# rockcarry/ffcnn

Measured on AMD Instinct MI355X. Metric: frames/sec yolo-fastest-1.1 @320x320 batch-64 per GPU (u8 BGR frames -> net_input's conversion in the first kernel -> full forward: conv stack + YOLO decode + NMS, boxes on rank 0), higher is better.
Workload: dtype f32

## Files before the change

### ffcnn_amd/capi.py

```python
import ctypes as C
import os
import subprocess

import numpy as np

HERE = os.path.dirname(os.path.abspath(__file__))
ROOT = os.path.dirname(HERE)
DATA = os.path.join(ROOT, "data")
CFG = os.path.join(DATA, "yolo-fastest-1.1.cfg")
WEIGHTS = os.path.join(DATA, "yolo-fastest-1.1.weights")

f32p = C.POINTER(C.c_float)


class FFGPU:
    MAX_DET = 128
    MERGE_LDS_SLOTS = 1024
    KEEP_ALL, COMPAT_V6, NO_GRAPH, NO_FUSE, HOST_DETS, SPLIT2, CONCURRENT, BF16_PW = 1, 2, 4, 8, 16, 32, 64, 128
    FEAT_FLAT, FEAT_MEAN, FEAT_MAX = 0, 1, 2
    POST_NONE, POST_SOFTMAX, POST_L2 = 0, 1, 2
    TOPK_MAX = 16
    RELABEL_KEEP_SCORE, RELABEL_LABEL_SCORE = 0, 1
    RELABEL_ENTRIES, RELABEL_MERGED = 0, 1
    K_AUTO, K_GENERIC, K_DW_STREAM, K_DW_LDS, K_PW_MFMA, K_PW_GEMM, _K6, K_DENSE_SMALL, K_IGEMM, K_PW_BF16, K_GROUP_THIN, K_PW_X3, K_CONV_X3, K_PW_X3T = range(14)
# ... 226 lines not shown
ZONES_EVENTS_HEADER = ("considered", "known", "fresh", "refused", "duplicate", "anonymous", "dropped", "freed", "live", "frame")
ZONES_STATE_HEADER = 144
TRACK_DETS = 128
TRACK_ENTRIES, TRACK_MERGED = 0, 1
TRACK_IDS_HEADER = ("considered", "matched", "born", "refused", "dropped", "freed", "live", "frame")
CROP_F32, CROP_U8 = 0, 1
CROP_ENTRIES, CROP_MERGED = 0, 1
REDACT_FILL, REDACT_MOSAIC = 0, 1
REDACT_OUTSIDE = 1
REDACT_ENTRIES, REDACT_MERGED = 0, 1
BLUR_OUTSIDE = 1
BLUR_ENTRIES, BLUR_MERGED = 0, 1
DRAW_ENTRIES, DRAW_MERGED = 0, 1
YUV_BT601_LIMITED, YUV_BT601_FULL, YUV_BT709_LIMITED, YUV_BT709_FULL = 0, 1, 2, 3

assert C.sizeof(LAYER) == 120 and C.sizeof(NET) == 104 and C.sizeof(BBOX) == 24
assert C.sizeof(FrameDets) == 16 + 24 * FFGPU.MAX_DET
assert C.sizeof(BgrFrame) == 24 and C.sizeof(Nv12Frame) == 40 and C.sizeof(Tile) == 16 and C.sizeof(TileRect) == 16
assert C.sizeof(DrawStyle) == 24 and C.sizeof(CropSpec) == 72 and C.sizeof(Crop) == 48
assert C.sizeof(TrackSpec) == 32 and C.sizeof(Track) == 48
assert C.sizeof(FeatureSpec) == 16 and C.sizeof(Label) == 8 and C.sizeof(RelabelSpec) == 16
assert C.sizeof(Gallery) == 40 and C.sizeof(RedactSpec) == 40 and C.sizeof(BlurSpec) == 40
assert C.sizeof(TextItem) == 64 and C.sizeof(CaptionSpec) == 48
assert C.sizeof(SegItem) == 32 and C.sizeof(OutlineSpec) == 40
assert C.sizeof(TrailPoint) == 12 and C.sizeof(TrailSlot) == 416 and C.sizeof(TrailsSpec) == 64
assert C.sizeof(HeatSpec) == 56 and C.sizeof(HeatBlendSpec) == 48
assert C.sizeof(MotionSpec) == 64
assert C.sizeof(Zone) == 96 and C.sizeof(Line) == 32 and C.sizeof(Scene) == 1040 and C.sizeof(ZonesSpec) == 32 and C.sizeof(ZoneSlot) == 64

BOX_DTYPE = np.dtype([("type", "<i4"), ("score", "<f4"), ("x1", "<f4"), ("y1", "<f4"), ("x2", "<f4"), ("y2", "<f4")])
DETS_DTYPE = np.dtype([("count", "<i4"), ("ncand", "<i4"), ("overflow", "<i4"), ("nfull", "<i4"),
                       ("box", BOX_DTYPE, (FFGPU.MAX_DET,))])
CROP_DTYPE = np.dtype([("target", "<i4"), ("box", "<i4"), ("type", "<i4"), ("score", "<f4"), ("x0", "<i4"), ("y0", "<i4"), ("w", "<i4"), ("h", "<i4"),
                       ("sw", "<i4"), ("sh", "<i4"), ("s1", "<i4"), ("s2", "<i4")])
TRACK_DTYPE = np.dtype([("id", "<i4"), ("type", "<i4"), ("score", "<f4"), ("x1", "<f4"), ("y1", "<f4"), ("x2", "<f4"), ("y2", "<f4"),
                        ("hits", "<i4"), ("missed", "<i4"), ("born", "<i4"), ("det", "<i4"), ("reserved", "<i4")])
ZONE_SLOT_DTYPE = np.dtype([("id", "<i4"), ("px", "<f4"), ("py", "<f4"), ("inside", "<i4"), ("last", "<i4"), ("reserved", "<i4", (3,)), ("since", "<i4", (8,))])
TRAIL_POINT_DTYPE = np.dtype([("x", "<i4"), ("y", "<i4"), ("frame", "<i4")])
TRAIL_SLOT_DTYPE = np.dtype([("id", "<i4"), ("last", "<i4"), ("n", "<i4"), ("head", "<i4"), ("cx", "<i4"), ("cy", "<i4"), ("reserved", "<i4", (2,)),
                             ("ring", TRAIL_POINT_DTYPE, (32,))])
LABEL_DTYPE = np.dtype([("index", "<i4"), ("value", "<f4")])
TEXT_ITEM_DTYPE = np.dtype([("x", "<i4"), ("y", "<i4"), ("fg", "u1", (4,)), ("bg", "u1", (4,)), ("scale", "u1"), ("flags", "u1"), ("len", "u1"), ("reserved", "u1"),
                            ("text", "u1", (44,))])
SEG_ITEM_DTYPE = np.dtype([("x0", "<i4"), ("y0", "<i4"), ("x1", "<i4"), ("y1", "<i4"), ("color", "u1", (4,)), ("thickness", "u1"), ("dash", "u1"), ("flags", "u1"),
                           ("reserved", "u1"), ("reserved2", "<i4", (2,))])

EXPORTS = ["net_load", "net_free", "net_input", "net_forward", "net_dump", "net_profile", "groupconv",
           "ffgpu_device_count", "ffgpu_set_device", "ffgpu_last_error", "ffgpu_build_info",
           "ffgpu_net_weights_dev", "ffgpu_net_weights_commit",
           "ffgpu_exec_create", "ffgpu_exec_destroy", "ffgpu_exec_batch", "ffgpu_exec_arena_bytes",
           "ffgpu_exec_kernel_count", "ffgpu_exec_work_model", "ffgpu_exec_set_scale", "ffgpu_exec_forward_dev", "ffgpu_exec_forward_host",
           "ffgpu_exec_forward_bgr_dev", "ffgpu_exec_forward_bgr_frames_dev", "ffgpu_exec_forward_nv12_frames_dev", "ffgpu_exec_dets_dev", "ffgpu_exec_dets_host", "ffgpu_exec_set_ring", "ffgpu_exec_set_ring_strided", "ffgpu_exec_read_dets", "ffgpu_exec_read_layer", "ffgpu_exec_hash_layers",
           "ffgpu_exec_read_boxes", "ffgpu_exec_cand_capacity", "ffgpu_exec_graph_captures",
           "ffgpu_exec_profile", "ffgpu_exec_profile_steps", "ffgpu_exec_step_model", "ffgpu_groupconv_dev", "ffgpu_groupconv_kernel_name", "ffgpu_groupconv_time_dev", "ffgpu_irb_dev", "ffgpu_irb_flags_dev", "ffgpu_irb_plan_text", "ffgpu_irb_thin_launch_text", "ffgpu_irb_s2_launch_text", "ffgpu_irb_stage_plan_text", "ffgpu_front_plan_text", "ffgpu_irb_instantiations", "ffgpu_knobs_text", "ffgpu_dwpw_dev", "ffgpu_packed_records_bytes", "ffgpu_pack_records", "ffgpu_unpack_records",
           "ffgpu_shard_range", "ffgpu_node_create", "ffgpu_node_destroy", "ffgpu_node_ndev", "ffgpu_node_shard", "ffgpu_node_set_scale",
           "ffgpu_node_input_dev", "ffgpu_node_input_slot_dev", "ffgpu_node_depth", "ffgpu_node_rccl_ranks", "ffgpu_node_forward", "ffgpu_node_forward_host",
           "ffgpu_node_submit", "ffgpu_node_wait", "ffgpu_node_run",
           "ffgpu_merge_tiles_scratch_bytes", "ffgpu_merge_tiles_dev", "ffgpu_exec_merge_tiles", "ffgpu_exec_merged_dev", "ffgpu_exec_read_merged",
           "ffgpu_exec_read_merged_boxes", "ffgpu_tile_plan",
           "ffgpu_draw_boxes_bgr_dev", "ffgpu_draw_boxes_nv12_dev", "ffgpu_exec_draw_bgr", "ffgpu_exec_draw_nv12",
           "ffgpu_crop_table_bytes", "ffgpu_crop_slot_bytes", "ffgpu_crop_boxes_bgr_dev", "ffgpu_crop_boxes_nv12_dev", "ffgpu_exec_crop_bgr", "ffgpu_exec_crop_nv12",
           "ffgpu_crops_to_source_dev",
           "ffgpu_track_state_bytes", "ffgpu_track_reset_dev", "ffgpu_track_boxes_dev", "ffgpu_exec_track",
           "ffgpu_feature_dim", "ffgpu_exec_feature_dim", "ffgpu_features_dev", "ffgpu_exec_features", "ffgpu_topk_dev", "ffgpu_crops_relabel_dev",
           "ffgpu_exec_relabel",
           "ffgpu_match_workspace_bytes", "ffgpu_match_dev", "ffgpu_gallery_enroll_dev",
           "ffgpu_redact_boxes_bgr_dev", "ffgpu_redact_boxes_nv12_dev", "ffgpu_exec_redact_bgr", "ffgpu_exec_redact_nv12",
           "ffgpu_blur_boxes_bgr_dev", "ffgpu_blur_boxes_nv12_dev", "ffgpu_exec_blur_bgr", "ffgpu_exec_blur_nv12",
           "ffgpu_zones_state_bytes", "ffgpu_scene_check", "ffgpu_zones_reset_dev", "ffgpu_zones_boxes_dev", "ffgpu_exec_zones",
           "ffgpu_font_builtin", "ffgpu_draw_text_bgr_dev", "ffgpu_draw_text_nv12_dev", "ffgpu_caption_boxes_dev", "ffgpu_exec_caption_bgr", "ffgpu_exec_caption_nv12",
           "ffgpu_caption_scene_dev",
           "ffgpu_draw_segments_bgr_dev", "ffgpu_draw_segments_nv12_dev", "ffgpu_outline_spec_check", "ffgpu_outline_scene_dev",
           "ffgpu_trails_state_bytes", "ffgpu_trails_spec_check", "ffgpu_trails_reset_dev", "ffgpu_trails_boxes_dev", "ffgpu_exec_trails",
           "ffgpu_heat_state_bytes", "ffgpu_heat_spec_check", "ffgpu_heat_blend_spec_check", "ffgpu_heat_palette", "ffgpu_heat_reset_dev", "ffgpu_heat_boxes_dev",
           "ffgpu_exec_heat", "ffgpu_heat_blend_bgr_dev", "ffgpu_heat_blend_nv12_dev",
           "ffgpu_motion_state_bytes", "ffgpu_motion_spec_check", "ffgpu_motion_reset_dev", "ffgpu_motion_update_bgr_dev", "ffgpu_motion_update_nv12_dev",
           "ffgpu_motion_gate_dev", "ffgpu_exec_motion_gate",
           "ffgpu_preview_spec_check", "ffgpu_preview_rect", "ffgpu_preview_grid", "ffgpu_preview_tile", "ffgpu_preview_bgr_dev", "ffgpu_preview_nv12_dev",
           "ffgpu_warp_spec_check", "ffgpu_warp_mesh_size", "ffgpu_warp_mesh_orient", "ffgpu_warp_mesh_homography", "ffgpu_warp_mesh_lens", "ffgpu_warp_point",
           "ffgpu_warp_tile", "ffgpu_warp_bgr_dev", "ffgpu_warp_nv12_dev"]
DIAG_EXPORTS = ["ffgpu_membench", "ffgpu_pipe_probe", "ffgpu_pipe_probe2", "ffgpu_pipe_probe3", "ffgpu_mfma_floor", "ffgpu_diag_x3_term", "ffgpu_diag_xl_op", "ffgpu_clock_probe"]


def library_path():
    return os.environ.get("FFCNN_HIP_LIB") or os.path.join(HERE, "lib", "libffcnn_hip.so")


def build_library(force=False):
    cmd = ["make", "-C", os.path.join(HERE, "csrc")]
    if force:
        subprocess.check_call(cmd + ["clean"], stdout=subprocess.DEVNULL)
    subprocess.check_call(cmd, stdout=subprocess.DEVNULL)
    return library_path()


_lib = None


def lib():
    global _lib
    if _lib is not None:
        return _lib
    path = library_path()
    if not os.path.exists(path):
        raise RuntimeError("%s is missing: run `python -c 'import __graft_entry__ as g; g.build()'` "
                           "(the HIP extension is the only compute path)" % path)
    L = C.CDLL(path)
    vp, i, sz = C.c_void_p, C.c_int, C.c_size_t
    L.net_load.restype = C.POINTER(NET)
    L.net_load.argtypes = [C.c_char_p, C.c_char_p, i, i]
    L.net_free.argtypes = [C.POINTER(NET)]
    L.net_input.argtypes = [C.POINTER(NET), vp, i, i, f32p, f32p]
    L.net_forward.argtypes = [C.POINTER(NET)]
    L.net_dump.argtypes = [C.POINTER(NET)]
    L.net_profile.argtypes = [C.POINTER(NET)]
    L.groupconv.argtypes = [f32p, f32p, f32p] + [i] * 12 + [C.POINTER(f32p), C.POINTER(i)]
    L.ffgpu_last_error.restype = C.c_char_p
    L.ffgpu_build_info.restype = C.c_char_p
    if b" DIAG " in L.ffgpu_build_info() and os.environ.get("FFCNN_HIP_ALLOW_DIAG") != "1":
        raise RuntimeError("%s is a DIAG (lab) build of libffcnn_hip; set FFCNN_HIP_ALLOW_DIAG=1 to load it on purpose" % path)
    L.ffgpu_set_device.argtypes = [i]
    L.ffgpu_net_weights_dev.argtypes = [C.POINTER(NET), C.POINTER(vp), C.POINTER(sz)]
    L.ffgpu_net_weights_commit.argtypes = [C.POINTER(NET), vp]
    L.ffgpu_exec_create.restype = vp
    L.ffgpu_exec_create.argtypes = [C.POINTER(NET), i, i]
    L.ffgpu_exec_destroy.argtypes = [vp]
    L.ffgpu_exec_batch.argtypes = [vp]
    L.ffgpu_exec_arena_bytes.restype = sz
    L.ffgpu_exec_arena_bytes.argtypes = [vp]
    L.ffgpu_exec_kernel_count.argtypes = [vp]
    L.ffgpu_exec_work_model.argtypes = [vp, C.POINTER(C.c_double), C.POINTER(C.c_double)]
    L.ffgpu_exec_set_scale.argtypes = [vp, i, i]
    L.ffgpu_exec_forward_dev.argtypes = [vp, vp, vp]
    L.ffgpu_exec_forward_host.argtypes = [vp, f32p]
    L.ffgpu_exec_forward_bgr_dev.argtypes = [vp, vp, i, i, f32p, f32p, vp]
    L.ffgpu_exec_forward_bgr_frames_dev.argtypes = [vp, C.POINTER(BgrFrame), i, f32p, f32p, vp]
    L.ffgpu_exec_forward_nv12_frames_dev.argtypes = [vp, C.POINTER(Nv12Frame), i, f32p, f32p, vp]
    L.ffgpu_exec_dets_dev.argtypes = [vp, C.POINTER(vp), C.POINTER(sz)]
    L.ffgpu_exec_dets_host.restype = vp; L.ffgpu_exec_dets_host.argtypes = [vp]
    L.ffgpu_exec_set_ring.argtypes = [vp, vp, C.c_int]
    L.ffgpu_exec_set_ring_strided.argtypes = [vp, vp, C.c_int, C.c_int]
    L.ffgpu_exec_read_dets.argtypes = [vp, vp, i]
    L.ffgpu_exec_read_layer.argtypes = [vp, i, i, f32p, sz]
    L.ffgpu_exec_hash_layers.argtypes = [vp, vp, i]
    L.ffgpu_exec_profile.argtypes = [vp, vp, f32p]
    L.ffgpu_exec_profile_steps.argtypes = [vp, vp, C.POINTER(i), f32p, i]
    L.ffgpu_exec_step_model.argtypes = [vp, C.POINTER(i), C.POINTER(C.c_double), i]
    L.ffgpu_groupconv_dev.argtypes = [vp, vp, vp] + [i] * 15 + [vp]
    L.ffgpu_groupconv_kernel_name.restype = C.c_char_p
    L.ffgpu_groupconv_kernel_name.argtypes = [i] * 10
    L.ffgpu_groupconv_time_dev.restype = C.c_float
    L.ffgpu_groupconv_time_dev.argtypes = [vp, vp, vp] + [i] * 17 + [vp]
    L.ffgpu_irb_dev.restype = C.c_float
    L.ffgpu_irb_dev.argtypes = [vp] * 6 + [i] * 13 + [vp]
    L.ffgpu_irb_flags_dev.restype = C.c_float
    L.ffgpu_irb_flags_dev.argtypes = [vp] * 6 + [i] * 14 + [vp]
    L.ffgpu_irb_thin_launch_text.argtypes = [i] * 12 + [C.c_char_p, i]
    L.ffgpu_irb_s2_launch_text.argtypes = [i] * 12 + [C.c_char_p, i]
    L.ffgpu_irb_plan_text.argtypes = [i] * 12 + [C.c_char_p, i]
    L.ffgpu_irb_stage_plan_text.argtypes = [i] * 7 + [C.c_char_p, i]
    L.ffgpu_front_plan_text.argtypes = [i] * 4 + [C.c_char_p, i]
    L.ffgpu_irb_instantiations.argtypes = [C.c_char_p, i]
    L.ffgpu_knobs_text.argtypes = [C.c_char_p, i]
    L.ffgpu_exec_read_boxes.argtypes = [vp, i, vp, i]
    L.ffgpu_exec_cand_capacity.argtypes = [vp]
    L.ffgpu_exec_graph_captures.argtypes = [vp]
    L.ffgpu_dwpw_dev.restype = C.c_float
    L.ffgpu_dwpw_dev.argtypes = [vp] * 4 + [i] * 10 + [vp]
    L.ffgpu_packed_records_bytes.restype = C.c_size_t
    L.ffgpu_packed_records_bytes.argtypes = [i, i]
    L.ffgpu_pack_records.restype = i
    L.ffgpu_pack_records.argtypes = [vp, i, C.c_long, i, i, vp, vp]
    L.ffgpu_shard_range.argtypes = [i, i, i, C.POINTER(i), C.POINTER(i)]
    L.ffgpu_shard_range.restype = None
    L.ffgpu_node_create.restype = vp
    L.ffgpu_node_create.argtypes = [C.POINTER(NET), i, C.POINTER(i), i, i, i]
    L.ffgpu_node_destroy.argtypes = [vp]
    L.ffgpu_node_ndev.argtypes = [vp]
    L.ffgpu_node_shard.argtypes = [vp, i, C.POINTER(i), C.POINTER(i), C.POINTER(i)]
    L.ffgpu_node_set_scale.argtypes = [vp, i, i]
    L.ffgpu_node_input_dev.restype = vp
    L.ffgpu_node_input_dev.argtypes = [vp, i]
    L.ffgpu_node_input_slot_dev.restype = vp
    L.ffgpu_node_input_slot_dev.argtypes = [vp, i, i]
    L.ffgpu_node_depth.argtypes = [vp]
    if hasattr(L, "ffgpu_node_rccl_ranks"):
        L.ffgpu_node_rccl_ranks.argtypes = [vp]
    L.ffgpu_node_submit.restype = C.c_long
    L.ffgpu_node_submit.argtypes = [vp, f32p]
    L.ffgpu_node_wait.argtypes = [vp, C.c_long, vp]
    L.ffgpu_node_run.argtypes = [vp, C.c_long, vp]
    L.ffgpu_unpack_records.argtypes = [vp, i, i, vp]
    L.ffgpu_node_forward.argtypes = [vp, vp]
    L.ffgpu_node_forward_host.argtypes = [vp, f32p, vp]
    L.ffgpu_merge_tiles_scratch_bytes.restype = sz
    L.ffgpu_merge_tiles_scratch_bytes.argtypes = [i, i]
    L.ffgpu_merge_tiles_dev.argtypes = [vp, vp, i, C.POINTER(Tile), i, i, C.c_float, i, vp, vp, vp, sz, vp]
    L.ffgpu_exec_merge_tiles.argtypes = [vp, C.POINTER(Tile), i, i, vp]
    L.ffgpu_exec_merged_dev.argtypes = [vp, C.POINTER(vp), C.POINTER(sz)]
    L.ffgpu_exec_read_merged.argtypes = [vp, vp, i]
    L.ffgpu_exec_read_merged_boxes.argtypes = [vp, i, vp, i]
    L.ffgpu_tile_plan.argtypes = [i] * 7 + [C.POINTER(TileRect), i]
    L.ffgpu_draw_boxes_bgr_dev.argtypes = [vp, vp, i, C.POINTER(i), C.POINTER(BgrFrame), i, C.POINTER(DrawStyle), vp]
    L.ffgpu_draw_boxes_nv12_dev.argtypes = [vp, vp, i, C.POINTER(i), C.POINTER(Nv12Frame), i, C.POINTER(DrawStyle), vp]
    L.ffgpu_exec_draw_bgr.argtypes = [vp, i, C.POINTER(BgrFrame), i, C.POINTER(DrawStyle), vp]
    L.ffgpu_exec_draw_nv12.argtypes = [vp, i, C.POINTER(Nv12Frame), i, C.POINTER(DrawStyle), vp]
    L.ffgpu_redact_boxes_bgr_dev.argtypes = [vp, vp, i, C.POINTER(i), C.POINTER(BgrFrame), i, C.POINTER(RedactSpec), vp]
    L.ffgpu_redact_boxes_nv12_dev.argtypes = [vp, vp, i, C.POINTER(i), C.POINTER(Nv12Frame), i, C.POINTER(RedactSpec), vp]
    L.ffgpu_exec_redact_bgr.argtypes = [vp, i, C.POINTER(BgrFrame), i, C.POINTER(RedactSpec), vp]
    L.ffgpu_exec_redact_nv12.argtypes = [vp, i, C.POINTER(Nv12Frame), i, C.POINTER(RedactSpec), vp]
    L.ffgpu_blur_boxes_bgr_dev.argtypes = [vp, vp, i, C.POINTER(i), C.POINTER(BgrFrame), C.POINTER(BgrFrame), i, C.POINTER(BlurSpec), vp]
# ... 1239 lines not shown


FRONT_FORMS = {"f32": 0, "u8": 1, "bgr_frames": 2, "nv12_frames": 3}


def front_plan_text(batch, pw, ph, form="f32"):
    buf = C.create_string_buffer(256)
    if lib().ffgpu_front_plan_text(batch, pw, ph, FRONT_FORMS[form], buf, len(buf)) < 0:
        raise RuntimeError("ffgpu_front_plan_text failed: %s" % last_error())
    return buf.value.decode()


def irb_instantiations():
    buf = C.create_string_buffer(4096)
    n = lib().ffgpu_irb_instantiations(buf, len(buf))
    if n < 0 or n >= len(buf):
        raise RuntimeError("ffgpu_irb_instantiations failed: %s" % (last_error() if n < 0 else "%d bytes" % n))
    return buf.value.decode().split()


def knobs():
    buf = C.create_string_buffer(1 << 16)
    n = lib().ffgpu_knobs_text(buf, len(buf))
    if n < 0 or n >= len(buf):
        raise RuntimeError("ffgpu_knobs_text failed: %s" % (last_error() if n < 0 else "%d bytes" % n))
    rows = []
    for line in buf.value.decode().splitlines():
        name, kind, dflt, cls, value, text = line.split(" ", 5)
        rows.append({"name": name, "kind": kind, "default": None if dflt == "-" else dflt if dflt == "computed" else int(dflt), "cls": cls, "value": value, "text": text})
    return rows


def dwpw_dev(d_in, d_wd, d_wp, d_out, batch, iw, ih, c, oc, fs, actd=2, actp=0, warmup=0, iters=0, stream=None):
    us = lib().ffgpu_dwpw_dev(d_in, d_wd, d_wp, d_out, batch, iw, ih, c, oc, fs, actd, actp, warmup, iters, stream)
    if us < 0:
        raise RuntimeError("ffgpu_dwpw_dev failed: %s" % last_error())
    return us


def irb_thin_launch_text(shape, flags=0):
    buf = C.create_string_buffer(256)
    if lib().ffgpu_irb_thin_launch_text(*shape, flags, buf, len(buf)) < 0:
        raise RuntimeError("ffgpu_irb_thin_launch_text failed: %s" % last_error())
    return buf.value.decode()


def irb_s2_launch_text(shape, flags=0):
    buf = C.create_string_buffer(256)
    if lib().ffgpu_irb_s2_launch_text(*shape, flags, buf, len(buf)) < 0:
        raise RuntimeError("ffgpu_irb_s2_launch_text failed: %s" % last_error())
    return buf.value.decode()


def irb_dev(d_in, d_w1, d_wd, d_w2, d_res, d_out, batch, iw, ih, ic, ec, oc, stride, act1=2, actd=2, act2=0, res_act=0,
            warmup=0, iters=0, stream=None, flags=0):
    us = lib().ffgpu_irb_flags_dev(d_in, d_w1, d_wd, d_w2, d_res, d_out, batch, iw, ih, ic, ec, oc, stride, act1, actd, act2, res_act, flags,
                                   warmup, iters, stream)
    if us < 0:
        raise RuntimeError("ffgpu_irb_dev failed: %s" % last_error())
    return us


def preview_pane(src=None, dst=None):
    p = PreviewPane()
    if src is not None:
        p.sx, p.sy, p.sw, p.sh = (int(v) for v in src)
    if dst is not None:
        p.dx, p.dy, p.dw, p.dh = (int(v) for v in dst)
    return p


def preview_spec(fit=PREVIEW_STRETCH, fill=(0, 0, 0), keep_bars=False):
    sp = PreviewSpec()
    sp.fit, sp.flags = fit, PREVIEW_KEEP_BARS if keep_bars else 0
    sp.fill[:] = (int(fill[0]), int(fill[1]), int(fill[2]), 0)
    return sp


def preview_spec_check(spec):
    _check(lib().ffgpu_preview_spec_check(spec), "ffgpu_preview_spec_check")


def preview_rect(src_w, src_h, dst_w, dst_h, pane, spec, nv12=False):
    out = (C.c_int * 8)()
    _check(lib().ffgpu_preview_rect(src_w, src_h, dst_w, dst_h, pane, spec, int(bool(nv12)), out), "ffgpu_preview_rect")
    return tuple(out)


def preview_grid(npanes, cols, dst_w, dst_h, gap=0, nv12=False):
    arr = (PreviewPane * max(1, npanes))()
    _check(lib().ffgpu_preview_grid(npanes, cols, dst_w, dst_h, gap, int(bool(nv12)), arr), "ffgpu_preview_grid")
    return [PreviewPane.from_buffer_copy(arr[k]) for k in range(npanes)]


def preview_tile():
    out = (C.c_int * 3)()
    _check(lib().ffgpu_preview_tile(out), "ffgpu_preview_tile")
    return tuple(out)


def _preview_panes(panes):
    arr = (PreviewPane * max(1, len(panes)))()
    for k, p in enumerate(panes):
        arr[k] = p
    return arr

# ... 101 lines not shown
```

### ffcnn_amd/csrc/ffgpu_conv_kernels.inc

```
#include "ffgpu_dw_stream.inc"
#include "ffgpu_pw_mfma.inc"
#include "ffgpu_pw_gemm32.inc"
#include "ffgpu_pw_bf16.inc"
#include "ffgpu_conv_igemm.inc"
#include "ffgpu_dwpw.inc"
#include "ffgpu_conv_dense.inc"
#include "ffgpu_irb.inc"
#include "ffgpu_irb_thin.inc"
#include "ffgpu_irb_thin_s2.inc"
#include "ffgpu_front.inc"
#include "ffgpu_irb_wave.inc"
#include "ffgpu_irb_wave2.inc"
#include "ffgpu_irb_stage.inc"
#include "ffgpu_pw_x3.inc"
#include "ffgpu_pw_x3t.inc"
#include "ffgpu_conv_x3.inc"
#include "ffgpu_dw_lds.inc"
#include "ffgpu_dw_pair.inc"
#include "ffgpu_conv_thin.inc"

struct BareScratch {
    float *p = nullptr; size_t n = 0; int dev = -1;
    float *get(size_t need)
    {
// ... 174 lines not shown
           d.out_ns == (long)d.ow * d.oh && d.out_cs == (long)d.N * d.ow * d.oh && (!d.residual || (d.res_ns == d.out_ns && d.res_cs == d.out_cs));
}
static int igemm_wm(const ConvDesc &d) { return d.oc / d.groups > 64 ? 2 : 1; }
static bool igemm_vec(const ConvDesc &d)
{
    return d.fs == 3 && d.stride == 1 && d.pad == 1 && d.ow >= 4 && d.iw == d.ow && d.ih == d.oh &&
           (long)d.N * d.oh * ((d.ow + 3) & ~3) < (1L << 31) && !knob(K_IGEMM_NOVEC);
}
static int igemm_kc(const ConvDesc &d) { return igemm_vec(d) ? (igemm_wm(d) == 1 ? IG_KC3N : IG_KC3) : IG_KC; }
static int igemm_split(const ConvDesc &d)
{
    if (d.nsplit > 0) return d.nsplit;
    const int f = knob(K_IGEMM_SPLIT);
    const int WM = d.oc / d.groups > 64 ? 2 : 1, TN = WM == 2 ? 128 : 256, kc = igemm_kc(d);
    const long P = (long)d.N * d.oh * (igemm_vec(d) ? (d.ow + 3) & ~3 : d.ow), tiles = ((P + TN - 1) / TN) * ((d.oc / d.groups + 64 * WM - 1) / (64 * WM)) * d.groups;
    const int nchunks = (d.fs * d.fs * (d.ic / d.groups) + kc - 1) / kc;
    int S = 1;
    const long slots = 768;
    while (S < 8 && tiles * (S + 1) <= slots && nchunks / (S + 1) >= 4) S++;
    if (f >= 1 && f <= 16) S = std::min(f, std::max(1, nchunks));
    return S;
}
static size_t igemm_part_floats(const ConvDesc &d) { const int S = igemm_split(d); return S > 1 ? (size_t)S * d.oc * d.N * d.oh * d.ow : 0; }
static void igemm_dims(const ConvDesc &d, int &WM, int &nchunks, int &ntm, int &img)
{
    WM = igemm_wm(d);
    const int kc = igemm_kc(d);
    nchunks = (d.fs * d.fs * (d.ic / d.groups) + kc - 1) / kc; ntm = (d.oc / d.groups + 64 * WM - 1) / (64 * WM);
    img = nchunks * (kc / 2) * WM * 128 + 2 * 64 * WM;
}

static bool ig_x3_ok(const ConvDesc &d)
{
    if (!(igemm_ok(d) && d.groups == 1 && !d.in_ind && !(d.flags & FFGPU_F_BATCH_INPUT) && d.ic >= 8 && d.ic % 8 == 0 && d.in_cs > 0 && d.in_ns > 0 &&
          (long)(d.ic + 32) * d.in_cs + (long)d.N * d.in_ns < (1L << 30))) return false;
    if (d.fs == 1)
        return d.stride == 1 && d.pad == 0 && conv_cnhw_contiguous(d) && ((long)d.N * d.ih * d.iw) % 4 == 0;
    if ((long)d.N * d.oh * ((d.ow + 3) & ~3) >= (1L << 31) - 64 || d.ow < 4) return false;
    if (d.fs == 3 && d.stride == 2 && d.pad == 1)
        return d.iw == 2 * d.ow && d.ih == 2 * d.oh && knob(K_IGX3_S2) != 0;
    return igemm_vec(d) && d.iw >= 4;
}
static int ig_x3_nw(const ConvDesc &d) { const int f = knob(K_IGX3_NW); return f == 8 || f == 4 ? f : (d.stride == 2 ? 8 : 4); }
static long ig_x3_npg(const ConvDesc &d) { const long ntn = ((long)d.N * d.oh * (d.fs == 1 ? d.ow : (d.ow + 3) & ~3) + 63) / 64; return (ntn + ig_x3_nw(d) - 1) / ig_x3_nw(d); }
static int ig_x3_mt_plan(const ConvDesc &d)
{
    const int f = knob(K_IGX3_MT);
    if (f == 4 || f == 2 || f == 1) return f;
    if (d.oc <= 32 || d.stride == 2) return d.oc <= 16 ? 1 : 2;
    return ig_x3_npg(d) * ((d.oc + 63) / 64) >= knob(K_IGX3_MT4_WGS) ? 4 : 2;
}
static int ig_x3_mt(const ConvDesc &d) { const int m = d.x3_mt == 4 || d.x3_mt == 2 || d.x3_mt == 1 ? d.x3_mt : ig_x3_mt_plan(d); return d.stride == 2 && m > 2 ? 2 : m; }
static void ig_x3_dims(const ConvDesc &d, int &MT, int &ngr, int &nrb, int &ntm) { MT = ig_x3_mt(d); ngr = (d.fs * (d.ic / 8) + 3) / 4; nrb = (d.oc + 15) / 16; ntm = (nrb + MT - 1) / MT; }
static size_t ig_x3_img_dwords(const ConvDesc &d) { int MT, ngr, nrb, ntm; ig_x3_dims(d, MT, ngr, nrb, ntm); return (size_t)ntm * ngr * 3 * d.fs * MT * 256; }
static bool ig_x3_auto(const ConvDesc &d)
{
    if (!ig_x3_ok(d)) return false;
    const int ntm = ((d.oc + 15) / 16 + ig_x3_mt_plan(d) - 1) / ig_x3_mt_plan(d);
    if (d.fs == 1)
        return knob(K_PW_X3S) != 0 && d.ic >= knob(K_PWX3S_MIN_IC) && d.oc >= knob(K_PWX3S_MIN_OC) &&
               ig_x3_npg(d) * ntm >= knob(K_PWX3S_MIN_WGS);
    if (knob(K_IG_X3) == 0) return false;
    return d.ic >= knob(K_IGX3_MIN_IC) && ig_x3_npg(d) * ntm >= knob(K_IGX3_MIN_WGS);
}
static int ig_x3_pack(const ConvDesc &d, float *pk, hipStream_t s)
{
    IgX3PackP q;
    int nrb;
    q.filt = d.filt; q.pk = reinterpret_cast<unsigned *>(pk); q.ic = d.ic; q.oc = d.oc; q.k4 = conv_k4(d); q.fs = d.fs;
    ig_x3_dims(d, q.MT, q.ngr, nrb, q.ntm);
    q.nunits = d.fs * (d.ic / 8);
    const long total = (long)ig_x3_img_dwords(d);
    hipLaunchKernelGGL(k_conv_x3_pack, dim3((unsigned)std::min((total + 255) / 256, 8192L)), dim3(256), 0, s, q);
    LAUNCH_OK("conv_x3_pack");
    return 0;
}

static int conv_pick(const ConvDesc &d, int variant)
{
    if (variant != FFGPU_K_AUTO) return variant;
    if (d.kernel) return d.kernel;
    if (knob(K_FORCE_GENERIC)) return FFGPU_K_GENERIC;
    if (dw_stream_ok(d)) return FFGPU_K_DW_STREAM;
    if (!(d.flags & FFGPU_BF16_PW) && pw_x3t_auto(d)) return FFGPU_K_PW_X3T;
    if (!(d.flags & FFGPU_BF16_PW) && d.fs == 1 && ig_x3_auto(d)) return FFGPU_K_CONV_X3;
    if (!(d.flags & FFGPU_BF16_PW) && pw_x3_auto(d)) return FFGPU_K_PW_X3;
    if ((d.flags & FFGPU_BF16_PW) && pw_gemm_ok(d) && d.oc >= 128 && d.ic >= 128 && (long)d.N * d.iw * d.ih >= 16384) return FFGPU_K_PW_BF16;
    if (pw_gemm_ok(d) && d.oc >= knob(K_PWG_MIN_OC) && d.ic >= knob(K_PWG_MIN_IC) && (long)d.N * d.iw * d.ih >= 16384 && !knob(K_NO_PW_GEMM)) return FFGPU_K_PW_GEMM;
    if (pw_mfma_ok(d)) return FFGPU_K_PW_MFMA;
    if (dw_lds_ok(d)) return FFGPU_K_DW_LDS;
    if (dense_small_ok(d)) return FFGPU_K_DENSE_SMALL;
    const bool igemm_on = !knob(K_NO_IGEMM);
    if (igemm_on && ig_x3_auto(d)) return FFGPU_K_CONV_X3;
    if (igemm_on && igemm_ok(d) && d.ic / d.groups >= 8) return FFGPU_K_IGEMM;
    if (group_thin_ok(d) && !knob(K_NO_GROUP_THIN)) return FFGPU_K_GROUP_THIN;
    return FFGPU_K_GENERIC;
}

void ffgpu_conv_plan(ConvDesc &d)
{
    d.kernel = 0; d.nsplit = 0; d.x3_mt = 0;
    const int k = conv_pick(d, FFGPU_K_AUTO);
    if (k == FFGPU_K_IGEMM) d.nsplit = igemm_split(d);
    if (k == FFGPU_K_CONV_X3) d.x3_mt = ig_x3_mt_plan(d);
    if (k == FFGPU_K_PW_X3T) d.x3_mt = pwx3t_rb_env();
    d.kernel = k;
}

template <int NV, int U, bool NT>
static void dw_stream_launch(const DwStreamP &p, hipStream_t s)
{
    const long blocks = (p.ntasks + 3) / 4;
    hipLaunchKernelGGL((k_dw3_stream<NV, U, NT>), dim3((unsigned)blocks), dim3(256), 0, s, p);
}

static int launch_dw_stream(const ConvDesc &d, const float *, hipStream_t s)
{
    const int U = knob(K_DW_U), BAND = knob(K_DW_BAND);
    const int nt_env = knob(K_DW_NT), NT = nt_env >= 0 ? nt_env : ((long)d.ic * d.N * d.iw * d.ih * 4 >= (128L << 20));
    DwStreamP p;
    p.in = d.in; p.filt = d.filt; p.out = d.out; p.residual = nullptr;
    p.W = d.iw; p.H = d.ih; p.planes = d.ic * d.N; p.N = d.N;
    p.lpr = d.iw / 4;
    const int NV = p.lpr > 64 ? 2 : 1;
    p.G = NV == 1 ? 64 / p.lpr : 1;
    const long pgroups = ((long)p.planes + p.G - 1) / p.G;
    int nb = BAND > 0 ? (d.ih + BAND - 1) / BAND : (int)((6144 + pgroups - 1) / pgroups);
// ... 239 lines not shown
    split_main_narrow(p.P, p.ntm, slots, knob(K_PWXT_NARROW) != 0, &ntn_main, &ntn_narrow);
    p.ntn = ntn_main;
    const long total = p.ntn * p.ntm;
    p.per_xcd = (int)((total + 7) / 8);
    p.nmain = 8 * p.per_xcd; p.tpw = 1;
    if (knob(K_PWXT_PERSIST) && total > slots) {
        p.nmain = slots / 8 * 8;
        p.tpw = (int)((8L * p.per_xcd + p.nmain - 1) / p.nmain);
    }
    p.dbg = knob(K_PWXT_DBG);
    { const int nt = knob(K_PWXT_NT); p.nt = nt >= 0 ? (nt != 0) : ((long)d.oc * p.P * 4 >= (128L << 20)); }
    const dim3 grid((unsigned)(p.nmain + ntn_narrow * p.ntm));
    p.dbg_t = nullptr;
#if XT_TRACE
    if (const char *tf = knob_text(K_PWXT_TRACE)) {
        const size_t nw = (size_t)((p.P + 31) / 32 + 4) * p.ntm * 8;
        unsigned long long *d_t = nullptr;
        if (hipMalloc(&d_t, nw * 8) != hipSuccess) return -1;
        (void)hipMemsetAsync(d_t, 0, nw * 8, s);
        p.dbg_t = d_t;
        if (RBv == 2) hipLaunchKernelGGL(k_pw_x3t<2>, grid, dim3(256), 0, s, p); else hipLaunchKernelGGL(k_pw_x3t<1>, grid, dim3(256), 0, s, p);
        (void)hipStreamSynchronize(s);
        std::vector<unsigned long long> h(nw);
        (void)hipMemcpy(h.data(), d_t, nw * 8, hipMemcpyDeviceToHost);
        (void)hipFree(d_t);
        if (FILE *fp = fopen(tf, "w")) {
            for (size_t i = 0; i < nw; i += 8) if (h[i]) fprintf(fp, "%llu %llu %llu %llu %llu %llu %llu\n", h[i], h[i + 1], h[i + 2], h[i + 3], h[i + 4], h[i + 5], h[i + 6]);
            fclose(fp);
        }
        return 0;
    }
#endif
    if (RBv == 2) hipLaunchKernelGGL(k_pw_x3t<2>, grid, dim3(256), 0, s, p);
    else          hipLaunchKernelGGL(k_pw_x3t<1>, grid, dim3(256), 0, s, p);
    LAUNCH_OK("pw_x3t");
    return 0;
}

static int launch_pw_bf16(const ConvDesc &d, const float *image, hipStream_t s)
{
    PwBf16P p;
    p.in = d.in; p.out = d.out; p.residual = d.residual;
    p.P = (long)d.N * d.iw * d.ih; p.ic = d.ic; p.oc = d.oc; p.act = d.act; p.res_act = d.res_act;
    pwbf16_dims(d, p.nchunks, p.ntm);
    p.img = p.nchunks * 2048 + 256;
    p.wpack = reinterpret_cast<const unsigned *>(image);
    p.ntn = (p.P + 127) / 128;
    p.per_xcd = (int)((p.ntn * p.ntm + 7) / 8);
    hipLaunchKernelGGL(k_pw_bf16, dim3((unsigned)(8 * p.per_xcd)), dim3(256), 0, s, p);
    LAUNCH_OK("pw_bf16");
    return 0;
}

static int launch_conv_x3(const ConvDesc &d, const float *image, hipStream_t s)
{
    IgX3P p;
    int MT;
    p.in = d.in; p.out = d.out; p.residual = d.residual; p.filt = d.filt;
    p.iw = d.iw; p.ih = d.ih; p.ow = d.ow; p.oh = d.oh; p.ic = d.ic; p.oc = d.oc; p.k4 = conv_k4(d); p.act = d.act; p.res_act = d.res_act;
    p.in_cs = (unsigned)d.in_cs; p.in_ns = (unsigned)d.in_ns;
    ig_x3_dims(d, MT, p.ngr, p.nrb, p.ntm);
    p.nunits = d.fs * (d.ic / 8);
    p.wpack = reinterpret_cast<const unsigned *>(image);
    const int NW = ig_x3_nw(d);
    p.owp = d.fs == 1 ? d.ow : (d.ow + 3) & ~3; p.P = (long)d.N * d.oh * d.ow; p.Pp = (long)d.N * d.oh * p.owp;
    p.ntn = (p.Pp + 63) / 64; p.npg = (p.ntn + NW - 1) / NW;
    const long nblk = 8 * (long)p.ntm * ((p.npg + 7) / 8);
    if (nblk > (1L << 30)) { ffgpu_set_error("conv_x3: too many tiles"); return -1; }
    const size_t lds = (size_t)2 * 3 * d.fs * MT * 1024 + (size_t)MT * 128;
    const dim3 grid((unsigned)nblk);
#define IGX3_LAUNCH(mt, nw, fs) do { if (lds_allow((const void *)k_conv_x3<mt, nw, fs>, lds, "conv_x3")) return -1; hipLaunchKernelGGL((k_conv_x3<mt, nw, fs>), grid, dim3(64 * nw), lds, s, p); } while (0)
#define IGX3_LAUNCH2(mt, nw) do { if (d.fs == 1) IGX3_LAUNCH(mt, nw, 1); else IGX3_LAUNCH(mt, nw, 3); } while (0)
    if (d.stride == 2) {
#define IGX3_LAUNCH_S2(mt, nw) do { if (lds_allow((const void *)k_conv_x3<mt, nw, 3, 2>, lds, "conv_x3")) return -1; hipLaunchKernelGGL((k_conv_x3<mt, nw, 3, 2>), grid, dim3(64 * nw), lds, s, p); } while (0)
        if (NW == 8) { if (MT == 2) IGX3_LAUNCH_S2(2, 8); else IGX3_LAUNCH_S2(1, 8); }
        else         { if (MT == 2) IGX3_LAUNCH_S2(2, 4); else IGX3_LAUNCH_S2(1, 4); }
#undef IGX3_LAUNCH_S2
    } else
    if (NW == 8) { if (MT == 4) IGX3_LAUNCH2(4, 8); else if (MT == 2) IGX3_LAUNCH2(2, 8); else IGX3_LAUNCH2(1, 8); }
    else         { if (MT == 4) IGX3_LAUNCH2(4, 4); else if (MT == 2) IGX3_LAUNCH2(2, 4); else IGX3_LAUNCH2(1, 4); }
#undef IGX3_LAUNCH2
#undef IGX3_LAUNCH
    LAUNCH_OK("conv_x3");
    return 0;
}

static int launch_igemm(const ConvDesc &d, const float *image, hipStream_t s)
{
    IgemmP p;
    int WM;
    const int gic = d.ic / d.groups, goc = d.oc / d.groups;
    p.in = d.in; p.in_ind = d.in_ind;
    p.P = (long)d.N * d.oh * d.ow; p.in_cs = d.in_cs; p.in_ns = d.in_ns;
    p.N = d.N; p.iw = d.iw; p.ih = d.ih; p.ic = gic; p.ow = d.ow; p.oh = d.oh; p.oc = goc; p.fs = d.fs; p.stride = d.stride; p.pad = d.pad;
    p.K = d.fs * d.fs * gic; p.act = d.act; p.res_act = d.res_act;
    igemm_dims(d, WM, p.nchunks, p.ntm, p.img);
    p.m_ff = umulhi_magic((long)d.fs * d.fs); p.m_f = umulhi_magic(d.fs);
    const size_t per_group = (size_t)p.img * p.ntm;
    p.nsplit = igemm_split(d);
    p.part = p.nsplit > 1 ? const_cast<float *>(image) + igemm_images_floats(d) : nullptr;
    const int TN = WM == 2 ? 128 : 256;
    p.owp = (d.ow + 3) & ~3; p.Pp = (long)d.N * d.oh * p.owp;
    p.ntn = ((igemm_vec(d) ? p.Pp : p.P) + TN - 1) / TN;
    const long total = p.ntn * p.ntm * p.nsplit * d.groups;
    if (total > (1L << 28)) { ffgpu_set_error("conv_igemm: too many tiles"); return -1; }
    p.per_xcd = (int)((total + 7) / 8);
    p.groups = d.groups; p.in_off = 0; p.g_in = (long)gic * d.in_cs; p.g_out = (long)goc * d.out_cs; p.g_w = (long)per_group;
    p.out = d.out; p.residual = d.residual; p.wpack = image;
    const dim3 grid((unsigned)(8 * p.per_xcd));
    if (igemm_vec(d)) {
        if (WM == 2)        hipLaunchKernelGGL((k_conv_igemm<2, true>), grid, dim3(256), 0, s, p);
        else if (goc <= 32) hipLaunchKernelGGL((k_conv_igemm<1, true, true>), grid, dim3(256), 0, s, p);
        else                hipLaunchKernelGGL((k_conv_igemm<1, true>), grid, dim3(256), 0, s, p);
    } else {
        if (WM == 2)        hipLaunchKernelGGL((k_conv_igemm<2, false>), grid, dim3(256), 0, s, p);
        else if (goc <= 32) hipLaunchKernelGGL((k_conv_igemm<1, false, true>), grid, dim3(256), 0, s, p);
        else                hipLaunchKernelGGL((k_conv_igemm<1, false>), grid, dim3(256), 0, s, p);
    }
    if (p.nsplit > 1) {
        IgemmRedP q;
        const int K = d.fs * d.fs * gic, k4 = (K + 3) & ~3;
        q.part = p.part; q.filt = d.filt; q.residual = d.residual; q.out = d.out; q.P = p.P; q.oc = d.oc; q.goc = goc;
        q.nsplit = p.nsplit; q.rl = k4 + 4; q.k4 = k4; q.act = d.act; q.res_act = d.res_act;
        hipLaunchKernelGGL(k_conv_igemm_reduce, dim3((unsigned)std::min(((long)d.oc * p.P + 255) / 256, 65536L)), dim3(256), 0, s, q);
    }
    LAUNCH_OK("conv_igemm");
    return 0;
}

static int launch_dw_lds(const ConvDesc &d, const float *, hipStream_t s)
{
    if (dw_pair_ok(d)) return launch_dw_pair(d, s);
    DwLdsP p;
    p.in = d.in; p.filt = d.filt; p.out = d.out;
    p.W = d.iw; p.H = d.ih; p.OW = d.ow; p.OH = d.oh; p.planes = d.ic * d.N; p.N = d.N;
    p.fs = d.fs; p.stride = d.stride; p.pad = d.pad; p.act = d.act; p.flags = d.flags; p.rowlen = conv_k4(d) + 4;
    p.LW = (((d.ow + 3) / 4 * 4 - 1) * d.stride + d.fs + 4 + 3) & ~3;
// ... 1018 lines not shown
```

### ffcnn_amd/csrc/ffgpu_conv_x3.inc

```
struct IgX3P {
    const float *in; float *out; const float *residual; const float *filt;
    const unsigned *wpack;
    long P, Pp;
    long ntn, npg;
    unsigned in_cs, in_ns;
    int  iw, ih, ow, oh, ic, oc, owp, k4;
    int  nunits, ngr;
    int  nrb, ntm;
    int  act, res_act;
};

struct IgX3PackP { const float *filt; unsigned *pk; int ic, oc, k4, nunits, ngr, ntm, MT, fs; };
__global__ void k_conv_x3_pack(IgX3PackP p)
{
    const int nkx = p.fs;
    const long total = (long)p.ntm * p.ngr * 3 * nkx * p.MT * 256;
    const int rl = p.k4 + 4;
    for (long i = (long)blockIdx.x * blockDim.x + threadIdx.x; i < total; i += (long)gridDim.x * blockDim.x) {
        const int d = (int)(i & 3), l = (int)((i >> 2) & 63);
        long t = i >> 8;
        const int part = (int)(t % 3); t /= 3;
        const int rb = (int)(t % p.MT); t /= p.MT;
        const int kx = (int)(t % nkx); t /= nkx;
        const int gr = (int)(t % p.ngr), mt = (int)(t / p.ngr);
        const int u = 4 * gr + (l >> 4), cb8 = u / nkx, ky = u - nkx * cb8;
        const int o = 16 * (mt * p.MT + rb) + (l & 15), c = u < p.nunits ? 8 * cb8 + 2 * d : p.ic;
        const float w0 = (o < p.oc && c < p.ic) ? p.filt[(long)o * rl + (c * nkx + ky) * nkx + kx] : 0.f;
        const float w1 = (o < p.oc && c + 1 < p.ic) ? p.filt[(long)o * rl + ((c + 1) * nkx + ky) * nkx + kx] : 0.f;
        p.pk[i] = irbw_x3_part(w0, part) | (irbw_x3_part(w1, part) << 16);
    }
}

template <int MT, int NW, int FS, int ST = 1>
__global__ void __launch_bounds__(64 * NW, 8 / NW) __attribute__((amdgpu_waves_per_eu(2))) k_conv_x3(IgX3P p)
{
    constexpr int NKX = FS, NCOL = FS == 1 ? 4 : (ST == 2 ? 9 : 6);
    constexpr int CH = 3 * NKX * MT * 256;
    typedef v4f_x3 v4a4 __attribute__((aligned(4)));
    typedef __attribute__((address_space(3))) void *lds_t;
    typedef const __attribute__((address_space(1))) void *glb_t;
    extern __shared__ __attribute__((aligned(16))) unsigned igx_lds[];
    const int tid = threadIdx.x, lane = tid & 63, wid = __builtin_amdgcn_readfirstlane(tid >> 6);
    const int kq = lane >> 4, n = lane & 15;
    const int xcd = (int)(blockIdx.x & 7);
    const long rr_ = (long)(blockIdx.x >> 3);
    const int mtile = (int)(rr_ % p.ntm);
    const long pg = (rr_ / p.ntm) * 8 + xcd;
    if (pg >= p.npg) return;
    const int rb0 = mtile * MT;
    float *sb = reinterpret_cast<float *>(igx_lds + 2 * CH);
    {
        const int rl = p.k4 + 4;
        for (int i = tid; i < MT * 32; i += 64 * NW) {
            const int o = 16 * rb0 + (i >> 1);
            sb[i] = o < p.oc ? p.filt[(long)o * rl + p.k4 + (i & 1)] : 0.f;
        }
    }

    const long pxt = pg * NW + wid;
    const long pq = pxt * 64 + 4 * n;
    const bool qvalid = pq < p.Pp;
    const unsigned pqu = (unsigned)(qvalid ? pq : 0);
    unsigned qn = 0; int qy = 0, qa = 0, qskip = 0;
    unsigned base_pix = pqu;
    bool okl = false, okr = false;
    if (FS == 3) {
        const unsigned plane = (unsigned)(p.oh * p.owp);
        qn = pqu / plane;
        const unsigned qrem = pqu - qn * plane;
        qy = (int)(qrem / (unsigned)p.owp);
        const int qx = (int)(qrem - (unsigned)qy * (unsigned)p.owp);
        qa = min(qx, p.ow - 4); qskip = qx - qa;
        base_pix = qvalid ? qn * p.in_ns + (unsigned)(ST * (qy * p.iw + qa)) : 0u;
        okl = qvalid && qa > 0; okr = ST == 1 && qvalid && qa + 4 < p.iw;
    }
    const int dl = okl ? -1 : 0, dr = okr ? 4 : 0;
    const gfp bsrc = to_global(p.in);

    v4f_x3 acc[MT][4];
#pragma unroll
    for (int t = 0; t < MT; t++)
#pragma unroll
        for (int q = 0; q < 4; q++) acc[t][q] = (v4f_x3){ 0.f, 0.f, 0.f, 0.f };

    v4f_x3 rc[8], rd[ST == 2 ? 8 : 1]; float rl_[8], rr[8];
    gfp bj[8];
#pragma unroll
    for (int j = 0; j < 8; j++) bj[j] = bsrc + (size_t)j * p.in_cs;
    auto unit_of = [&](int gr, unsigned &off0, bool &ok) {
        const unsigned u = (unsigned)min(4 * gr + kq, p.nunits - 1);
        const bool real = 4 * gr + kq < p.nunits;
        if (FS == 3) {
            const unsigned cb8 = __umulhi(u, 0x55555556u);
            const int ky = (int)(u - 3u * cb8);
            ok = real && qvalid && (unsigned)(ST * qy + ky - 1) < (unsigned)p.ih;
            off0 = 8u * cb8 * p.in_cs + (ok ? base_pix + (unsigned)((ky - 1) * p.iw) : base_pix);
        } else {
            ok = real && qvalid;
            off0 = 8u * u * p.in_cs + base_pix;
        }
    };
    auto issue = [&](int j, unsigned off0) {
        rc[j] = gld<v4a4>(bj[j] + off0);
        if (FS == 3) {
            rl_[j] = *(bj[j] + (off0 + (unsigned)dl));
            if (ST == 2) rd[j] = gld<v4a4>(bj[j] + (off0 + 4u));
            else rr[j] = *(bj[j] + (off0 + (unsigned)dr));
        }
    };
    constexpr int NP = (3 * NKX * MT + NW - 1) / NW;
    auto glds1 = [&](int gr, int i, auto BUF) {
        constexpr int buf = decltype(BUF)::value;
        const unsigned *src = p.wpack + ((size_t)mtile * p.ngr + gr) * CH;
        const int pc = wid + NW * i;
// ... 63 lines not shown
        const unsigned *A = igx_lds + buf * CH + lane * 4;
        u4_x3 a[3], an[3];
#pragma unroll
        for (int pt = 0; pt < 3; pt++) a[pt] = *reinterpret_cast<const u4_x3 *>(A + pt * 256);
#pragma unroll
        for (int kx = 0; kx < NKX; kx++)
#pragma unroll
            for (int t = 0; t < MT; t++) {
                const int nx = kx * MT + t + 1;
                if (!last) {
                    constexpr int NB = NKX * MT, PB = (4 + NB - 1) / NB, GB = (NP + NB - 1) / NB;
                    const int b = nx - 1;
                    __builtin_amdgcn_sched_barrier(0);
#pragma unroll
                    for (int d = b * PB; d < (b + 1) * PB; d++) if (d < 4) { issue(2 * d, noff0); issue(2 * d + 1, noff0); }
#pragma unroll
                    for (int i = b * GB; i < (b + 1) * GB; i++) if (i < NP) glds1(gr + 1, i, std::integral_constant<int, buf ^ 1>{});
                    __builtin_amdgcn_sched_barrier(0);
                }
                if (nx < NKX * MT) {
#pragma unroll
                    for (int pt = 0; pt < 3; pt++) an[pt] = *reinterpret_cast<const u4_x3 *>(A + (nx * 3 + pt) * 256);
                }
                constexpr int WP[6] = { 0, 1, 2, 0, 1, 0 }, XP[6] = { 2, 1, 0, 1, 0, 0 };
#pragma unroll
                for (int m = 0; m < 6; m++) {
                    const v8bf_x3 Af = __builtin_bit_cast(v8bf_x3, a[WP[m]]);
#pragma unroll
                    for (int q = 0; q < 4; q++)
                        acc[t][q] = __builtin_amdgcn_mfma_f32_16x16x32_bf16(Af, __builtin_bit_cast(v8bf_x3, pk[ST * q + kx][XP[m]]), acc[t][q], 0, 0, 0);
                }
                if (nx < NKX * MT) {
#pragma unroll
                    for (int pt = 0; pt < 3; pt++) a[pt] = an[pt];
                }
            }
        rowok = nrowok;
        __builtin_amdgcn_sched_barrier(0);
        if (!last) {
            __builtin_amdgcn_s_waitcnt(0x0f70);
            __syncthreads();
        }
    };
    {
        const std::integral_constant<int, 0> B0; const std::integral_constant<int, 1> B1;
        const std::false_type F; const std::true_type T;
        int gr = 0;
        for (; gr + 2 < p.ngr; gr += 2) { group(gr, B0, F); group(gr + 1, B1, F); }
        if (gr + 1 < p.ngr) { group(gr, B0, F); group(gr + 1, B1, T); }
        else group(gr, B0, T);
    }

    if (!qvalid) return;
    const float slope = p.act == 2 ? 0.1f : (p.act == 1 ? 0.f : 1.f), rslope = p.res_act == 2 ? 0.1f : (p.res_act == 1 ? 0.f : 1.f);
    const long px = FS == 3 ? ((long)qn * p.oh + qy) * p.ow + qa : pq;
    const bool vec = FS == 1 || (p.owp == p.ow && (p.P & 3) == 0);
#pragma unroll
    for (int t = 0; t < MT; t++)
#pragma unroll
        for (int r = 0; r < 4; r++) {
            const int o = 16 * (rb0 + t) + 4 * kq + r;
            if (o < p.oc) {
                const float sc = sb[2 * (16 * t + 4 * kq + r)], bi = sb[2 * (16 * t + 4 * kq + r) + 1];
                v4f_pw v = pw_fma4_apart(acc[t][0][r], acc[t][1][r], acc[t][2][r], acc[t][3][r], sc, bi);
                v = pw_act4(v, slope, p.act == 3);
                const long off = (long)o * p.P + px;
                if (vec) {
                    if (p.residual) {
                        const v4f_pw q4 = *reinterpret_cast<const v4f_pw *>(p.residual + off);
                        v = pw_act4(v + q4, rslope, p.res_act == 3);
                    }
                    *reinterpret_cast<v4f_pw *>(p.out + off) = v;
                } else {
                    if (p.residual) {
                        v4f_pw q4 = { 0.f, 0.f, 0.f, 0.f };
#pragma unroll
                        for (int q = 0; q < 4; q++) if (q >= qskip) q4[q] = p.residual[off + q];
                        v = pw_act4(v + q4, rslope, p.res_act == 3);
                    }
#pragma unroll
                    for (int q = 0; q < 4; q++) if (q >= qskip) p.out[off + q] = v[q];
                }
            }
        }
}
```

### ffcnn_amd/csrc/ffgpu_dev.hpp

```cpp
#pragma once
#include <hip/hip_runtime.h>
#include <stddef.h>
#include <stdint.h>
#include <vector>
#include "ffgpu_internal.h"
#include "ffgpu_args.hpp"
#include "ffgpu_streams_host.hpp"
#include "ffgpu_track_host.hpp"
#include "ffgpu_zones_host.hpp"
#include "ffgpu_text_host.hpp"
#include "ffgpu_lines_host.hpp"
#include "ffgpu_trails_host.hpp"
#include "ffgpu_heat_host.hpp"
#include "ffgpu_motion_host.hpp"
#include "ffgpu_preview_host.hpp"
#include "ffgpu_warp_host.hpp"

#define FFGPU_CHECK(expr)                                                                   \
    do {                                                                                    \
        hipError_t e_ = (expr);                                                             \
        if (e_ != hipSuccess) {                                                             \
            ffgpu_set_error("%s failed: %s (%s:%d)", #expr, hipGetErrorString(e_), __FILE__, __LINE__); \
            return -1;                                                                      \
        }                                                                                   \
    } while (0)

struct ConvDesc {
    const float *in;
    const float *const *in_ind;
    const float *filt;
    float       *out;
    const float *residual;
    const float *wpack;
    int   N;
    int   iw, ih, ic;
    int   ow, oh, oc;
    int   fs, stride, pad, groups;
    int   act;
    int   res_act;
    int   flags;
    long  in_cs, in_ns, out_cs, out_ns, res_cs, res_ns;
    int   nsplit;
    int   kernel;
    int   x3_mt;
};
#define FFGPU_F_BATCH_INPUT (1 << 30)

static inline int conv_k4(const ConvDesc &d) { return (d.fs * d.fs * (d.ic / d.groups) + 3) & ~3; }

enum { IRB_NONE = 0, IRB_THIN, IRB_WAVE, IRB_WG };
struct IrbPlan {
    int family;
    int inst;
    int half;
    int pack_floats;
    int lds, grid, block;
    int KS1, OT, NSI, NSO, TWq, TH, EW, EH, ngroups, G, WPB, big, x3, xl;
    int xcd, region;
    int TW, NF, ECH, NW, KS, wbufs, red_off;
    int band, front_band;
};
struct IrbDesc {
    const float *in; float *out; const float *residual;
    const float *w1, *wd, *w2;
    int N, H, W, OH, OW, ic, ec, oc, stride;
    int act1, actd, act2, res_act;
    const float *pk;
    int flags;
    IrbPlan plan;
};
bool   ffgpu_irb_plan(IrbDesc &d);
size_t ffgpu_irb_pack_floats(const IrbDesc &d);
int    ffgpu_irb_pack(const IrbDesc &d, float *pk, hipStream_t s);
int    ffgpu_launch_irb(const IrbDesc &d, hipStream_t s);
int    ffgpu_irb_plan_line(const IrbDesc &d, char *buf, size_t cap);
int    ffgpu_irb_thin_launch_line(const IrbDesc &d, char *buf, size_t cap);
int    ffgpu_irb_s2_launch_line(const IrbDesc &d, char *buf, size_t cap);
int    ffgpu_irb_keys(char *buf, size_t cap);
#define IRBS_MAXB 8
bool   ffgpu_irb_stage_ok(const IrbDesc *blocks, int B);
int    ffgpu_launch_irb_stage(const IrbDesc *blocks, int B, hipStream_t s);
int    ffgpu_irb_stage_line(const IrbDesc *blocks, int B, bool wanted, char *buf, size_t cap);
bool   ffgpu_front_ok(const ConvDesc &c, const IrbDesc &d);
enum InputForm { IN_F32, IN_U8, IN_BGR_FRAMES, IN_NV12_FRAMES, IN_FORMS };
int    ffgpu_launch_front(const ConvDesc &c, const IrbDesc &d, InputForm form, hipStream_t s);
bool   ffgpu_front_nv12_fused();
int    ffgpu_front_plan_line(const IrbDesc &d, InputForm form, char *buf, size_t cap);
int    ffgpu_front_nc(const IrbDesc &d);

bool   ffgpu_dwpw_ok(const ConvDesc &dw, const ConvDesc &pw);
size_t ffgpu_dwpw_pack_floats(const ConvDesc &dw, const ConvDesc &pw);
int    ffgpu_dwpw_pack(const ConvDesc &dw, const ConvDesc &pw, float *pk, hipStream_t s);
int    ffgpu_launch_dwpw(const ConvDesc &dw, const ConvDesc &pw, const float *wpack, hipStream_t s);

size_t ffgpu_pw_pack_floats(const ConvDesc &d);
void   ffgpu_conv_plan(ConvDesc &d);
int    ffgpu_pw_pack(const ConvDesc &d, float *pk, hipStream_t s);

#define FFGPU_YUV_MATRICES { { 16, 298, 409, 100, 208, 516 }, { 0, 256, 359, 88, 183, 454 }, { 16, 298, 459, 55, 136, 541 }, { 0, 256, 403, 48, 120, 475 } }
int  ffgpu_launch_set_frames(FrameDesc *d_tab, const FrameDesc *h_desc, int n, hipStream_t s);
int  ffgpu_launch_input_frames(const FrameDesc *d_tab, bool nv12, float *out, int N, int W, int H, const float mean[3], const float norm[3], hipStream_t s);

struct ExecParams {
    const float *frames;
    int s1, s2;
    ffgpu_frame_dets *ring;
    int ring_slots, ring_stride;
    int bbox_max;
    const unsigned char *bgr;
    long  bgr_frame;
    int   bgr_pitch;
    float mean[3], norm[3];
    const FrameDesc *frames_tab;
};
int  ffgpu_launch_set_params(ExecParams *d_prm, const ExecParams &v, hipStream_t s);
bool ffgpu_conv_supports_ind(const ConvDesc &d);

bool ffgpu_no_device(const char *what);

int         ffgpu_launch_conv(const ConvDesc &d, int variant, hipStream_t s);
const char *ffgpu_conv_kernel_name(const ConvDesc &d, int variant);
int ffgpu_launch_pool(const float *in, float *out, int N, int c, int w, int h, int fs, int stride, int is_max, hipStream_t s);
int ffgpu_launch_spp(const float *in, float *const out[3], const int fs[3], int n, long planes, int w, int h, hipStream_t s);
int ffgpu_launch_upsample(const float *in, float *out, long planes, int w, int h, int stride, hipStream_t s);
int ffgpu_launch_add_act(const float *a, const float *b, float *out, long n, int act, hipStream_t s);
int ffgpu_launch_copy(const float *src, float *dst, long n, hipStream_t s);
int ffgpu_launch_hash64(const float *x, long n, unsigned long long *out, hipStream_t s);
int ffgpu_launch_input_bgr(const unsigned char *bgr, float *out, int N, int w, int h, int W, int H,
                           int sw, int sh, int s1, int s2, const float mean[3], const float norm[3], hipStream_t s);

struct YoloHead {
    const float *in;
    int   w, h, classes;
    int   anchors[3][2];
    float thresh, scale_xy;
    int   key_base;
};
int ffgpu_launch_yolo(const YoloHead &hd, int N, int netw, int neth, BBOX *cand, int *cand_key, int *ncand, int cap, int *ring_ctr, hipStream_t s);
int ffgpu_launch_nms(const BBOX *cand, const int *cand_key, int *ncand, int cap, BBOX *full, void *scratch,
                     ffgpu_frame_dets *dets, ffgpu_frame_dets *dets_host, const int *ring_ctr, int N,
                     float thresh, int use_min, const ExecParams *prm, hipStream_t s);
#define FFGPU_NMS_LDS_CAP 8192
bool ffgpu_nms_in_lds(int cap_pow2);
int ffgpu_launch_clear(int *ncand, int N, int *ring_ctr, hipStream_t s);

int    ffgpu_merge_build_tab(const char *what, const ffgpu_tile *tiles, int ntiles, int nimages, std::vector<int> &tab, std::vector<int> *off);
size_t ffgpu_merge_tab_bytes(int ntiles);
int    ffgpu_launch_set_ints(int *d_dst, const int *h_src, int n, hipStream_t s);
int    ffgpu_launch_merge_tiles(const int *d_tab, const std::vector<int> &tab, const ffgpu_frame_dets *recs, const BBOX *lists, int stride,
                                float thresh, int use_min, ffgpu_frame_dets *out_recs, BBOX *out_lists, void *scratch, hipStream_t s);

int ffgpu_draw_style_check(const char *what, const ffgpu_draw_style *st, unsigned pal[256], int *npal);
int ffgpu_launch_draw(bool nv12, const DetSource &src, const std::vector<DrawTarget> &targets, const unsigned pal[256], int npal, int thickness, hipStream_t s);

struct CropPlan {
    int   out_w, out_h, form, per_target, nclasses, num, den;
    float min_score, mean[3], norm[3];
    unsigned char classes[256];
};
int ffgpu_box_sel_check(const char *what, int nclasses, const unsigned char *classes, int margin_num, int margin_den);
int ffgpu_crop_spec_check(const char *what, const ffgpu_crop_spec *sp, CropPlan &pl);
int ffgpu_crop_buffers_check(const char *what, const void *d_out, const void *d_table, int capacity);
int ffgpu_launch_crop(bool nv12, const DetSource &src, const std::vector<CropSrc> &sources, const CropPlan &pl, void *d_out, void *d_table, int capacity, hipStream_t s);

struct RedactPlan {
    int   mode, cell, outside, nclasses, num, den;
    float min_score;
    unsigned colour;
    unsigned char classes[256];
};
int ffgpu_redact_spec_check(const char *what, const ffgpu_redact_spec *sp, bool nv12, RedactPlan &pl);
int ffgpu_launch_redact(const char *what, bool nv12, const DetSource &src, const std::vector<DrawTarget> &targets, const RedactPlan &pl, hipStream_t s);

struct BlurPlan {
    int   radius, passes, outside, nclasses, num, den;
    float min_score;
    unsigned char classes[256];
};
int ffgpu_blur_spec_check(const char *what, const ffgpu_blur_spec *sp, BlurPlan &pl);
int ffgpu_launch_blur(const char *what, bool nv12, const DetSource &src, const std::vector<DrawTarget> &targets, const std::vector<DrawTarget> &scratch,
                      const BlurPlan &pl, hipStream_t s);

int ffgpu_state_reset(const char *what, void *d_state, size_t all, int nstreams, int which_stream, void *stream);

int ffgpu_launch_track(const DetSource &src, const int *streams, int ntargets, const ffgpu_track_spec &spec, void *d_state, void *d_ids, void *d_out_records, void *d_out_lists, hipStream_t s);

int ffgpu_launch_zones(const DetSource &src, const int *streams, int ntargets, const ffgpu_zones_spec &spec, const void *d_scenes, void *d_state, const void *d_ids,
                       void *d_events, void *d_out_records, void *d_out_lists, hipStream_t s);

int ffgpu_launch_draw_text(bool nv12, const void *d_items, int items_stride, const void *d_font, const std::vector<DrawTarget> &targets, hipStream_t s);
int ffgpu_launch_caption_boxes(const DetSource &src, int ntargets, const CaptionPlan &pl, const void *d_ids, void *d_items, int items_stride, hipStream_t s);
// ... 18 lines not shown
```

### ffcnn_amd/csrc/ffgpu_exec.hip

```cpp
#include <algorithm>
#include <cstdarg>
#include <cstdint>
#include <cstdio>
#include <cstdlib>
#include <cstring>
#include <map>
#include <mutex>
#include <string>
#include <type_traits>
#include <vector>

#include "ffgpu_dev.hpp"
#include "ffgpu_knobs.hpp"
#include "ffgpu_plan.hpp"
#include "conv.h"

static thread_local char g_err[512] = "";

extern "C" void ffgpu_set_error(const char *fmt, ...)
{
    va_list ap;
    va_start(ap, fmt);
    vsnprintf(g_err, sizeof g_err, fmt, ap);
    va_end(ap);
// ... 67 lines not shown
{
    if (bytes == 0) return 0;
    if (pinned_ours(h_src, bytes)) { FFGPU_CHECK(hipMemcpy(d_dst, h_src, bytes, hipMemcpyHostToDevice)); return 0; }
    Bounce &bn = bounce_cur();
    std::lock_guard<std::mutex> lk(bn.mu);
    if (bounce_ready(bn)) return -1;
    char *const g_bounce = bn.p;
    for (size_t off = 0; off < bytes; off += BOUNCE_BYTES) {
        const size_t n = std::min(BOUNCE_BYTES, bytes - off);
        memcpy(g_bounce, static_cast<const char *>(h_src) + off, n);
        FFGPU_CHECK(hipMemcpy(static_cast<char *>(d_dst) + off, g_bounce, n, hipMemcpyHostToDevice));
    }
    return 0;
}

static int copy_d2h(void *h_dst, const void *d_src, size_t bytes)
{
    if (bytes == 0) return 0;
    if (pinned_ours(h_dst, bytes)) { FFGPU_CHECK(hipMemcpy(h_dst, d_src, bytes, hipMemcpyDeviceToHost)); return 0; }
    Bounce &bn = bounce_cur();
    std::lock_guard<std::mutex> lk(bn.mu);
    if (bounce_ready(bn)) return -1;
    char *const g_bounce = bn.p;
    for (size_t off = 0; off < bytes; off += BOUNCE_BYTES) {
        const size_t n = std::min(BOUNCE_BYTES, bytes - off);
        FFGPU_CHECK(hipMemcpy(g_bounce, static_cast<const char *>(d_src) + off, n, hipMemcpyDeviceToHost));
        memcpy(static_cast<char *>(h_dst) + off, g_bounce, n);
    }
    return 0;
}

#define FFGPU_INTERNAL_CHILD 0x40000000

enum StepKind { S_CONV, S_POOL, S_UPSAMPLE, S_ADD, S_COPY, S_YOLO, S_NMS, S_CLEAR, S_TOCNHW, S_IRB, S_FRONT, S_DWPW, S_STAGE };

struct Step {
    StepKind kind;
    int      layer;
    int      ltype;
    ConvDesc conv;
    ConvDesc conv2;
    bool     in_is_input;
    bool     b_is_input;
    const float *a, *b;
    float   *out;
    long     n;
    int      w, h, c, fs, stride, flag;
    YoloHead head;
    IrbDesc  irb;
    std::vector<IrbDesc> run;
    float   *out2[2];
    int      fs2[2];
    int      lane;
};

struct ffgpu_netdev {
    NET   *net = nullptr;
    std::mutex mu;
    std::vector<ffgpu_exec *> execs;
    double us_acc[LAYER_TYPE_TOTOAL] = {};
    float *d_weights = nullptr;
    size_t weight_bytes = 0;
    int    device = 0;
    ffgpu_exec *exec1 = nullptr;
};

struct InputSrc {
    InputForm form;
    const float *frames;
    const unsigned char *bgr; long bgr_frame; int bgr_pitch;
    const FrameDesc *ftab;
    float mean[3], norm[3];
    InputSrc slice(int c, int part_frames, size_t part_floats) const
    {
        InputSrc p = *this;
        if (frames) p.frames = frames + c * part_floats;
        if (bgr) p.bgr = bgr + (long)c * part_frames * bgr_frame;
        if (ftab) p.ftab = ftab + (size_t)c * part_frames;
        return p;
    }
};
static InputSrc fp32_src(const float *d_frames) { InputSrc in = {}; in.frames = d_frames; return in; }
static InputSrc u8_src(InputForm form, const float mean[3], const float norm[3])
{
    InputSrc in = {};
    in.form = form;
    for (int k = 0; k < 3; k++) { in.mean[k] = mean[k]; in.norm[k] = norm[k]; }
    return in;
}

struct ffgpu_exec {
    NET *net = nullptr;
    ffgpu_netdev *dev = nullptr;
    int  N = 1, flags = 0, device = 0;
    int  in_c = 0, in_h = 0, in_w = 0;
    std::vector<Step>   steps;
    NetLayout layout;
    float *arena = nullptr;
    float *d_input = nullptr;
    float *d_pack = nullptr;
    BBOX  *d_cand = nullptr;
    int   *d_cand_key = nullptr, *d_ncand = nullptr;
    int    cand_cap = 1, bbox_max = 1;
    BBOX  *d_full = nullptr;
    void  *d_nms_scratch = nullptr;
    ExecParams *d_prm = nullptr;
    bool   indirect = false;
    ExecParams prm_sent = {}; hipStream_t prm_stream = nullptr; bool prm_valid = false;
    InputSrc last = {};
    ffgpu_frame_dets *d_dets = nullptr;
    ffgpu_frame_dets *h_dets = nullptr, *h_dets_dev = nullptr;
    FrameDesc *d_ftab = nullptr;
    std::vector<FrameDesc> ftab_sent; hipStream_t ftab_stream = nullptr;
    float *h_stage = nullptr;
    ffgpu_frame_dets *d_merged = nullptr; BBOX *d_merged_full = nullptr; void *d_merge_scratch = nullptr; int *d_mtab = nullptr;
    std::vector<int> mtab_sent, mrg_off; hipStream_t mtab_stream = nullptr;
    ffgpu_frame_dets *ring = nullptr; int ring_slots = 0; int *d_ringctr = nullptr;
    int ring_stride = 0;
    static constexpr int MAXPART = 8;
    ffgpu_exec *child[MAXPART] = {};
    int nchild = 0;
    hipStream_t part_stream[MAXPART] = {}; hipEvent_t part_ev[MAXPART] = {};
    bool is_child = false;
    int    s1 = 1, s2 = 1;
    hipStream_t own_stream = nullptr, last_stream = nullptr;
    hipStream_t side_stream = nullptr;
    hipEvent_t  ev_fork = nullptr, ev_join = nullptr;
    hipGraphExec_t graph[IN_FORMS] = {};
    struct Keyed { const float *in; hipGraphExec_t g; unsigned long stamp; };
    std::vector<Keyed> graphs;
    unsigned long graph_stamp = 0;
    int captures = 0;
    int kernel_count = 0;
};

static float *tensor_ptr(const ffgpu_exec *ex, int t) { return ex->arena + ex->layout.offset_of(t); }

static bool stage_wanted(int N, int flags)
{
    return (flags & FFGPU_CONCURRENT) && !(flags & (FFGPU_KEEP_ALL | FFGPU_NO_FUSE)) && N >= 32 && knob(K_IRB_STAGE) != 0;
}

static PlanOptions plan_options(const ffgpu_exec *ex)
{
    PlanOptions o;
    o.batch = ex->N;
    o.keep_all = ex->flags & FFGPU_KEEP_ALL;
    o.fuse = !(ex->flags & FFGPU_NO_FUSE);
    o.branch = knob(K_BRANCH) && !ex->is_child;
    o.no_irb = knob(K_NO_IRB); o.irb_min_ec = knob(K_IRB_MIN_EC);
    o.dwpw = knob(K_DWPW);
    o.stage = stage_wanted(ex->N, ex->flags);
    return o;
// ... 161 lines not shown
                cp.a = ptr(t); cp.out = ptr(i) + off; cp.n = (long)o.w * o.h * o.c * N;
                S.push_back(cp);
                off += cp.n;
            }
            break; }
        case LAYER_TYPE_YOLO: {
            st.kind = S_YOLO;
            YoloHead &hd = st.head;
            hd.in = in_ptr(i, &from_input);
            if (from_input) { ffgpu_set_error("yolo head directly on the input is not supported"); return -1; }
            hd.w = a.w; hd.h = a.h; hd.classes = a.class_num;
            memcpy(hd.anchors, a.anchor_list, sizeof hd.anchors);
            hd.thresh = a.ignore_thres; hd.scale_xy = a.scale_x_y; hd.key_base = key_base;
            key_base += a.w * a.h * 3;
            S.push_back(st);
            break; }
        default: break;
        }
    }
    if (bad_chain) { ffgpu_set_error("a layer consumes the (non-existent) output of a yolo head"); return -1; }
    return 0;
}

static void fuse_front(ffgpu_exec *ex)
{
    std::vector<Step> &S = ex->steps;
    for (size_t k = 0; k + 1 < S.size(); k++) {
        Step &c0 = S[k];
        const Step &b0 = S[k + 1];
        if (c0.kind != S_CONV || b0.kind != S_IRB || c0.layer < 0 || ex->layout.nuses[c0.layer] != 1) continue;
        if (!ffgpu_front_ok(c0.conv, b0.irb)) continue;
        c0.kind = S_FRONT; c0.irb = b0.irb;
        ex->layout.readable[c0.layer] = 0;
        S.erase(S.begin() + k + 1);
        break;
    }
}

static void merge_spp(std::vector<Step> &S)
{
    for (size_t i = 0; i + 1 < S.size(); i++) {
        Step &a = S[i];
        if (a.kind != S_POOL || !a.flag || a.stride != 1 || a.in_is_input || (long)a.w * a.h > 8192) continue;
        int k = 0;
        while (k < 2 && i + 1 < S.size()) {
            const Step &b = S[i + 1];
            if (b.kind != S_POOL || !b.flag || b.stride != 1 || b.in_is_input || b.a != a.a || b.c != a.c || b.w != a.w || b.h != a.h) break;
            a.out2[k] = b.out; a.fs2[k] = b.fs; k++;
            S.erase(S.begin() + i + 1);
        }
    }
}

static void rewrite_steps(ffgpu_exec *ex)
{
    std::vector<Step> &S = ex->steps;
    const bool fuse = !(ex->flags & FFGPU_NO_FUSE);
    if (fuse) { fuse_front(ex); merge_spp(S); }
    const auto head = std::find_if(S.begin(), S.end(), [](const Step &t) { return t.kind == S_YOLO; });
    if (head != S.end() && fuse) {
        head->flag = 1;
        S.erase(std::remove_if(S.begin(), S.end(), [](const Step &t) { return t.kind == S_CLEAR; }), S.end());
    }
    { Step nm{}; nm.kind = S_NMS; nm.layer = -1; nm.ltype = LAYER_TYPE_YOLO; S.push_back(nm); }
    const NetLayout &nl = ex->layout;
    for (Step &st : S) st.lane = (nl.side_lo >= 0 && st.layer >= nl.side_lo && st.layer <= nl.side_hi) ? 1 : 0;
}

static size_t pack_floats(const Step &st)
{
    if (st.kind == S_IRB) return ffgpu_irb_pack_floats(st.irb);
    if (st.kind == S_STAGE) { size_t n = 0; for (const IrbDesc &d : st.run) n += ffgpu_irb_pack_floats(d); return n; }
    if (st.kind == S_DWPW) return ffgpu_dwpw_pack_floats(st.conv, st.conv2);
    if (st.kind == S_CONV) return ffgpu_pw_pack_floats(st.conv);
    return 0;
}

static int place_constants(ffgpu_exec *ex)
{
    size_t tot = 0;
    for (Step &st : ex->steps) {
        if (st.kind == S_CONV) {
            if (st.in_is_input) st.conv.flags |= FFGPU_F_BATCH_INPUT;
            ffgpu_conv_plan(st.conv);
        }
        tot += pack_floats(st);
    }
    if (!tot) return 0;
    if (hipMalloc(&ex->d_pack, tot * sizeof(float)) != hipSuccess) { ffgpu_set_error("hipMalloc(pack) failed"); return -1; }
    size_t off = 0;
    for (Step &st : ex->steps) {
        const size_t n = pack_floats(st);
        if (st.kind == S_IRB) st.irb.pk = ex->d_pack + off;
        else if (st.kind == S_STAGE) { size_t o = off; for (IrbDesc &d : st.run) { d.pk = ex->d_pack + o; o += ffgpu_irb_pack_floats(d); } }
        else if (st.kind == S_DWPW) st.conv2.wpack = ex->d_pack + off;
        else if (st.kind == S_CONV && n) st.conv.wpack = ex->d_pack + off;
        off += n;
    }
    return 0;
}

static void decide_indirect(ffgpu_exec *ex)
{
    ex->indirect = !knob(K_NO_INDIRECT);
    for (const Step &st : ex->steps)
        if (st.b_is_input || (st.in_is_input && !(st.kind == S_FRONT || (st.kind == S_CONV && ffgpu_conv_supports_ind(st.conv))))) ex->indirect = false;
    if (ex->indirect)
        for (Step &st : ex->steps) if (st.in_is_input) st.conv.in_ind = reinterpret_cast<const float *const *>(ex->d_prm);
}

static int plan(ffgpu_exec *ex)
{
    std::vector<IrbDesc> irb_planned;
    if (plan_layout(ex, irb_planned) || plan_arena(ex) || plan_steps(ex, irb_planned)) return -1;
    rewrite_steps(ex);
    if (place_constants(ex)) return -1;
    decide_indirect(ex);
    ex->kernel_count = (int)ex->steps.size();
    return 0;
}

static int repack(ffgpu_exec *ex, hipStream_t s)
{
    for (const Step &st : ex->steps) {
        if (st.kind == S_IRB && ffgpu_irb_pack(st.irb, const_cast<float *>(st.irb.pk), s)) return -1;
        if (st.kind == S_STAGE) for (const IrbDesc &d : st.run) if (ffgpu_irb_pack(d, const_cast<float *>(d.pk), s)) return -1;
        if (st.kind == S_DWPW && ffgpu_dwpw_pack(st.conv, st.conv2, const_cast<float *>(st.conv2.wpack), s)) return -1;
        if (st.kind == S_CONV && st.conv.wpack && ffgpu_pw_pack(st.conv, const_cast<float *>(st.conv.wpack), s)) return -1;
    }
    return 0;
}

static int issue_step(ffgpu_exec *ex, const Step &st, const InputSrc &in, hipStream_t s)
{
    const float *const d_frames = in.frames;
#ifdef FFGPU_DIAG
    if (knob_text(K_DBG_SKIP) || knob_text(K_DBG_KEEP)) {
        static bool warned = false;
        if (!warned) { warned = true; fprintf(stderr, "libffcnn_hip: FFGPU_DBG_SKIP / FFGPU_DBG_KEEP set -- launches are being dropped, RESULTS ARE WRONG (tuning only)\n"); }
    }
    if (const char *sk = knob_text(K_DBG_SKIP)) {
        int lo = -1, hi = -1;
        if (sscanf(sk, "%d:%d", &lo, &hi) == 2 && st.layer >= lo && st.layer <= hi && st.kind != S_NMS) return 0;
    }
    if (const char *sk = knob_text(K_DBG_KEEP)) {
        int lo = -1, hi = -1;
        if (sscanf(sk, "%d:%d", &lo, &hi) == 2 && (st.layer < lo || st.layer > hi) && st.kind != S_NMS) return 0;
    }
#endif
    switch (st.kind) {
    case S_CLEAR:
        return ffgpu_launch_clear(ex->d_ncand, ex->N, ex->d_ringctr, s);
    case S_CONV: {
        ConvDesc d = st.conv;
        if (st.in_is_input && !d.in_ind) d.in = d_frames;
        return ffgpu_launch_conv(d, FFGPU_K_AUTO, s); }
    case S_POOL:
        if (st.fs2[0]) {
            float *const outs[3] = { st.out, st.out2[0], st.out2[1] };
            const int fss[3] = { st.fs, st.fs2[0], st.fs2[1] };
            return ffgpu_launch_spp(st.a, outs, fss, st.fs2[1] ? 3 : 2, (long)ex->N * st.c, st.w, st.h, s);
        }
        return ffgpu_launch_pool(st.in_is_input ? d_frames : st.a, st.out, ex->N, st.c, st.w, st.h, st.fs, st.stride, st.flag, s);
    case S_UPSAMPLE:
        return ffgpu_launch_upsample(st.in_is_input ? d_frames : st.a, st.out, (long)ex->N * st.c, st.w, st.h, st.stride, s);
    case S_ADD:
        return ffgpu_launch_add_act(st.in_is_input ? d_frames : st.a, st.b_is_input ? d_frames : st.b, st.out, st.n, st.flag, s);
    case S_COPY:
        return ffgpu_launch_copy(st.a, st.out, st.n, s);
    case S_TOCNHW: {
        const long plane = (long)st.w * st.h;
        for (int c = 0; c < st.c; c++)
            FFGPU_CHECK(hipMemcpy2DAsync(st.out + (long)c * ex->N * plane, plane * sizeof(float),
                                         d_frames + (long)c * plane, (size_t)st.c * plane * sizeof(float),
                                         plane * sizeof(float), ex->N, hipMemcpyDeviceToDevice, s));
        return 0; }
    case S_IRB:
        return ffgpu_launch_irb(st.irb, s);
    case S_STAGE:
        return ffgpu_launch_irb_stage(st.run.data(), (int)st.run.size(), s);
    case S_DWPW:
        return ffgpu_launch_dwpw(st.conv, st.conv2, st.conv2.wpack, s);
    case S_FRONT: {
        ConvDesc d = st.conv;
        if (st.in_is_input && !d.in_ind) d.in = d_frames;
        return ffgpu_launch_front(d, st.irb, in.form, s); }
    case S_YOLO:
        return ffgpu_launch_yolo(st.head, ex->N, ex->in_w, ex->in_h, ex->d_cand, ex->d_cand_key, ex->d_ncand, ex->cand_cap,
                                 st.flag ? ex->d_ringctr : nullptr, s);
    case S_NMS:
        return ffgpu_launch_nms(ex->d_cand, ex->d_cand_key, ex->d_ncand, ex->cand_cap, ex->d_full, ex->d_nms_scratch,
                                ex->d_dets, ex->h_dets_dev, ex->d_ringctr, ex->N, 0.5f, 1, ex->d_prm, s);
    }
    return -1;
}

static int issue_all(ffgpu_exec *ex, const InputSrc &in, hipStream_t s)
{
    bool forked = false, joined = true;
    for (const Step &st : ex->steps) {
        if (st.lane == 1) {
            if (!ex->side_stream) FFGPU_CHECK(hipStreamCreateWithFlags(&ex->side_stream, hipStreamNonBlocking));
            if (!forked) {
                FFGPU_CHECK(hipEventRecord(ex->ev_fork, s));
                FFGPU_CHECK(hipStreamWaitEvent(ex->side_stream, ex->ev_fork, 0));
                forked = true; joined = false;
            }
            if (issue_step(ex, st, in, ex->side_stream) != 0) return -1;
            continue;
        }
        if (st.kind == S_NMS && !joined) {
            FFGPU_CHECK(hipEventRecord(ex->ev_join, ex->side_stream));
            FFGPU_CHECK(hipStreamWaitEvent(s, ex->ev_join, 0));
            joined = true;
        }
        if (issue_step(ex, st, in, s) != 0) return -1;
    }
    if (!joined) {
        FFGPU_CHECK(hipEventRecord(ex->ev_join, ex->side_stream));
        FFGPU_CHECK(hipStreamWaitEvent(s, ex->ev_join, 0));
    }
    return 0;
}

static int issue_split(ffgpu_exec *ex, const InputSrc &in, hipStream_t s)
{
    const int pn = ex->child[0]->N;
    const size_t part = (size_t)pn * ex->in_c * ex->in_h * ex->in_w;
    FFGPU_CHECK(hipEventRecord(ex->ev_fork, s));
    for (int c = 1; c < ex->nchild; c++) FFGPU_CHECK(hipStreamWaitEvent(ex->part_stream[c], ex->ev_fork, 0));
    for (int c = 0; c < ex->nchild; c++)
        if (issue_all(ex->child[c], in.slice(c, pn, part), c ? ex->part_stream[c] : s) != 0) return -1;
    for (int c = 1; c < ex->nchild; c++) {
        FFGPU_CHECK(hipEventRecord(ex->part_ev[c], ex->part_stream[c]));
        FFGPU_CHECK(hipStreamWaitEvent(s, ex->part_ev[c], 0));
    }
    return 0;
}

static int push_params(ffgpu_exec *ex, const InputSrc &in, hipStream_t s)
{
    if (ex->child[0]) {
// ... 161 lines not shown
          && hipHostGetDevicePointer((void **)&ex->h_dets_dev, ex->h_dets, 0) == hipSuccess;
        if (ok) memset(ex->h_dets, 0, sizeof(ffgpu_frame_dets) * (size_t)batch);
    }
    if (!ok) { ffgpu_set_error("executor buffers: %s", hipGetErrorString(hipGetLastError())); ffgpu_exec_destroy(ex); return nullptr; }
    ex->last_stream = ex->own_stream;
    if (split) {
        int K = 2;
        const int parts = knob(K_SPLIT_PARTS);
        if ((parts == 4 || parts == 8) && batch % parts == 0) K = parts;
        for (int c = 0; c < K; c++) {
            ffgpu_exec *ch = exec_create_on(dev, net, batch / K, (flags & ~FFGPU_HOST_DETS) | FFGPU_INTERNAL_CHILD);
            if (!ch) { ffgpu_exec_destroy(ex); return nullptr; }
            (void)hipFree(ch->d_dets); (void)hipFree(ch->d_full);
            ch->d_dets = ex->d_dets + (size_t)c * (batch / K);
            ch->d_full = ex->d_full + (size_t)c * (batch / K) * ex->cand_cap;
            ch->h_dets_dev = ex->h_dets_dev ? ex->h_dets_dev + (size_t)c * (batch / K) : nullptr;
            ex->child[c] = ch; ex->nchild = c + 1;
            ex->kernel_count += ch->kernel_count;
            ex->layout.arena_floats += ch->layout.arena_floats;
            if (c && (hipStreamCreateWithFlags(&ex->part_stream[c], hipStreamNonBlocking) != hipSuccess ||
                      hipEventCreateWithFlags(&ex->part_ev[c], hipEventDisableTiming) != hipSuccess)) {
                ffgpu_set_error("split executor: stream / event creation failed"); ffgpu_exec_destroy(ex); return nullptr; }
        }
        { std::lock_guard<std::mutex> lk(dev->mu); dev->execs.push_back(ex); }
        if (capture_at_create(ex)) { ffgpu_exec_destroy(ex); return nullptr; }
        return ex;
    }
    if (plan(ex) != 0 || repack(ex, ex->own_stream) != 0 || hipStreamSynchronize(ex->own_stream) != hipSuccess) { ffgpu_exec_destroy(ex); return nullptr; }
    { std::lock_guard<std::mutex> lk(dev->mu); dev->execs.push_back(ex); }
    if (!as_child && capture_at_create(ex)) { ffgpu_exec_destroy(ex); return nullptr; }
    return ex;
}

extern "C" void ffgpu_exec_destroy(ffgpu_exec *ex)
{
    if (!ex) return;
    int cur_dev = ex->device;
    (void)hipGetDevice(&cur_dev);
    if (cur_dev != ex->device) (void)hipSetDevice(ex->device);
    if (ex->last_stream) (void)hipStreamSynchronize(ex->last_stream);
    if (!ex->is_child) (void)hipDeviceSynchronize();
    for (int c = 0; c < ffgpu_exec::MAXPART; c++) {
        if (ex->child[c]) { ffgpu_exec_destroy(ex->child[c]); ex->child[c] = nullptr; }
        if (ex->part_stream[c]) (void)hipStreamDestroy(ex->part_stream[c]);
        if (ex->part_ev[c]) (void)hipEventDestroy(ex->part_ev[c]);
    }
    if (ex->is_child) { ex->d_dets = nullptr; ex->d_full = nullptr; }
    if (ex->dev) {
        std::lock_guard<std::mutex> lk(ex->dev->mu);
        ex->dev->execs.erase(std::remove(ex->dev->execs.begin(), ex->dev->execs.end(), ex), ex->dev->execs.end());
    }
    drop_graphs(ex);
    for (const Step &st : ex->steps) if (st.kind == S_TOCNHW) (void)hipFree(st.out);
    (void)hipFree(ex->arena); (void)hipFree(ex->d_input); (void)hipFree(ex->d_pack); (void)hipFree(ex->d_cand);
    (void)hipFree(ex->d_cand_key); (void)hipFree(ex->d_ncand); (void)hipFree(ex->d_dets);
    (void)hipFree(ex->d_full); (void)hipFree(ex->d_prm); (void)hipFree(ex->d_nms_scratch); (void)hipFree(ex->d_ftab);
    (void)hipFree(ex->d_merged); (void)hipFree(ex->d_merged_full); (void)hipFree(ex->d_merge_scratch); (void)hipFree(ex->d_mtab);
    if (ex->h_dets) (void)hipHostFree(ex->h_dets);
    if (ex->h_stage) (void)hipHostFree(ex->h_stage);
    (void)hipFree(ex->d_ringctr);
    if (ex->own_stream) (void)hipStreamDestroy(ex->own_stream);
    if (ex->side_stream) (void)hipStreamDestroy(ex->side_stream);
    if (ex->ev_fork) (void)hipEventDestroy(ex->ev_fork);
    if (ex->ev_join) (void)hipEventDestroy(ex->ev_join);
    if (cur_dev != ex->device) (void)hipSetDevice(cur_dev);
    delete ex;
}

extern "C" int ffgpu_exec_batch(const ffgpu_exec *ex) { return ex ? ex->N : 0; }
extern "C" size_t ffgpu_exec_arena_bytes(const ffgpu_exec *ex) { return ex ? ex->layout.arena_floats * sizeof(float) : 0; }
extern "C" int ffgpu_exec_kernel_count(const ffgpu_exec *ex) { return ex ? ex->kernel_count : 0; }

static double step_model_bytes(const ffgpu_exec *ex, const Step &st)
{
    const double N = ex->N;
    auto rows = [](const ConvDesc &d) { return (double)d.oc * (conv_k4(d) + 4); };
    switch (st.kind) {
    case S_CONV: { const ConvDesc &d = st.conv;
        return 4.0 * (N * d.ic * d.ih * d.iw + N * d.oc * d.oh * d.ow * (d.residual ? 2 : 1) + rows(d)); }
    case S_IRB: { const IrbDesc &d = st.irb;
        return 4.0 * (N * d.ic * d.H * d.W + N * d.oc * d.OH * d.OW * (d.residual ? 2 : 1) + (double)d.ec * (d.ic + 4 + 16) + (double)d.oc * (d.ec + 4)); }
    case S_STAGE: { const IrbDesc &d = st.run.front();
        return 4.0 * (N * d.ic * d.H * d.W + N * d.oc * d.OH * d.OW + (double)st.run.size() * ((double)d.ec * (d.ic + 4 + 16) + (double)d.oc * (d.ec + 4))); }
    case S_DWPW: { const ConvDesc &a = st.conv, &b = st.conv2;
        return 4.0 * (N * a.ic * a.ih * a.iw + N * b.oc * b.oh * b.ow + rows(a) + rows(b)); }
    case S_FRONT: { const ConvDesc &c = st.conv; const IrbDesc &d = st.irb;
        return 4.0 * (N * c.ic * c.ih * c.iw + N * d.oc * d.OH * d.OW + rows(c)); }
    case S_POOL: { const int np = 1 + (st.fs2[0] != 0) + (st.fs2[1] != 0);
        return 4.0 * N * st.c * ((double)st.w * st.h + (double)np * (st.w / st.stride) * (st.h / st.stride)); }
    case S_UPSAMPLE: return 4.0 * N * st.c * (double)st.w * st.h * (1 + st.stride * st.stride);
    case S_ADD: return 4.0 * 3 * st.n;
    case S_COPY: return 4.0 * 2 * st.n;
    case S_TOCNHW: return 4.0 * 2 * N * st.c * (double)st.w * st.h;
    case S_YOLO: return 4.0 * N * 3 * (5 + st.head.classes) * (double)st.head.w * st.head.h;
    default: return 0.0;
    }
}

extern "C" int ffgpu_exec_step_model(const ffgpu_exec *ex, int *layer_of, double *hbm_bytes, int cap)
{
    if (!ex || !ex->net || !layer_of || !hbm_bytes) { ffgpu_set_error("step_model: bad argument"); return -1; }
    if (ex->child[0]) { ffgpu_set_error("step_model: not available on a split executor"); return -1; }
    const int n = (int)std::min<size_t>(ex->steps.size(), (size_t)(cap > 0 ? cap : 0));
    for (int i = 0; i < n; i++) { layer_of[i] = ex->steps[i].layer; hbm_bytes[i] = step_model_bytes(ex, ex->steps[i]); }
    return n;
}

// ... 557 lines not shown
{
    if (!alive(ex, "hash_layers")) return -1;
    if (ex->child[0]) { ffgpu_set_error("hash_layers: not for FFGPU_SPLIT2 executors"); return -1; }
    if (!(ex->flags & FFGPU_KEEP_ALL)) { ffgpu_set_error("hash_layers needs an FFGPU_KEEP_ALL executor"); return -1; }
    const int L = ex->net->layer_num;
    if (!host_out || cap < L) { ffgpu_set_error("hash_layers: room for %d values needed", L); return -1; }
    unsigned long long *d = nullptr;
    FFGPU_CHECK(hipMalloc(&d, sizeof(unsigned long long) * L));
    hipStream_t s = ex->last_stream;
    int rc = 0, nh = 0;
    if (hipMemsetAsync(d, 0, sizeof(unsigned long long) * L, s) != hipSuccess) rc = -1;
    for (int i = 0; i < L && !rc; i++) {
        if (ex->layout.canon[i] < 0 || !ex->layout.readable[i]) continue;
        const LAYER &o = ex->net->layer_list[i + 1];
        if (ffgpu_launch_hash64(tensor_ptr(ex, ex->layout.canon[i]), (long)o.c * ex->N * o.w * o.h, d + i, s)) rc = -1;
        nh++;
    }
    if (!rc && hipStreamSynchronize(s) != hipSuccess) rc = -1;
    if (!rc && copy_d2h(host_out, d, sizeof(unsigned long long) * L)) rc = -1;
    (void)hipFree(d);
    if (rc) { ffgpu_set_error("hash_layers: a device call failed"); return -1; }
    return nh;
}

extern "C" int ffgpu_exec_read_layer(ffgpu_exec *ex, int layer, int frame, float *host_out, size_t cap_floats)
{
    if (!alive(ex, "read_layer")) return -1;
    if (!host_out || frame < 0 || frame >= ex->N) { ffgpu_set_error("read_layer: bad arguments"); return -1; }
    if (ex->child[0]) return ffgpu_exec_read_layer(ex->child[frame / ex->child[0]->N], layer, frame % ex->child[0]->N, host_out, cap_floats);
    FFGPU_CHECK(hipStreamSynchronize(ex->last_stream));
    if (layer == -2) {
        int cnt = 0;
        if (copy_d2h(&cnt, &ex->d_dets[frame].ncand, sizeof(int))) return -1;
        cnt = std::min(cnt, ex->cand_cap);
        if ((size_t)cnt * 6 > cap_floats) { ffgpu_set_error("read_layer: buffer too small"); return -1; }
        std::vector<BBOX> b(cnt);
        std::vector<int> k(cnt), idx(cnt);
        if (cnt) {
            if (copy_d2h(b.data(), ex->d_cand + (size_t)frame * ex->cand_cap, sizeof(BBOX) * cnt)) return -1;
            if (copy_d2h(k.data(), ex->d_cand_key + (size_t)frame * ex->cand_cap, sizeof(int) * cnt)) return -1;
        }
        for (int i = 0; i < cnt; i++) idx[i] = i;
        std::sort(idx.begin(), idx.end(), [&](int a, int c) { return k[a] < k[c]; });
        for (int i = 0; i < cnt; i++) memcpy(host_out + 6 * i, &b[idx[i]], sizeof(BBOX));
        return cnt;
    }
    if (layer == -1) {
        const size_t fl = (size_t)ex->in_c * ex->in_h * ex->in_w;
        if (ex->last.form != IN_F32) { ffgpu_set_error("read_layer: the last forward's frames were u8 images converted by the first kernel -- no fp32 input tensor exists"); return -1; }
        if (!ex->last.frames) { ffgpu_set_error("read_layer: no forward has run yet"); return -1; }
        if (fl > cap_floats) { ffgpu_set_error("read_layer: buffer too small"); return -1; }
        if (copy_d2h(host_out, ex->last.frames + (size_t)frame * fl, fl * sizeof(float))) return -1;
        return (int)fl;
    }
    if (!(ex->flags & FFGPU_KEEP_ALL)) { ffgpu_set_error("read_layer needs an FFGPU_KEEP_ALL executor"); return -1; }
    if (layer < 0 || layer >= ex->net->layer_num || ex->layout.canon[layer] < 0 || !ex->layout.readable[layer]) {
        ffgpu_set_error("read_layer: layer %d is not materialised by this executor (fused away or no tensor)", layer);
        return -1;
    }
    const LAYER &o = ex->net->layer_list[layer + 1];
    const size_t plane = (size_t)o.w * o.h;
    if (plane * o.c > cap_floats) { ffgpu_set_error("read_layer: buffer too small"); return -1; }
    const float *src = tensor_ptr(ex, ex->layout.canon[layer]) + (size_t)frame * plane;
    {
        const size_t row = plane * sizeof(float), per = std::max<size_t>(1, BOUNCE_BYTES / row);
        if (row > BOUNCE_BYTES) {
            for (size_t c = 0; c < (size_t)o.c; c++)
                if (copy_d2h(host_out + c * plane, src + c * plane * ex->N, row)) return -1;
            return (int)(plane * o.c);
        }
        Bounce &bn = bounce_cur();
        std::lock_guard<std::mutex> lk(bn.mu);
        if (bounce_ready(bn)) return -1;
        char *const g_bounce = bn.p;
        for (size_t c0 = 0; c0 < (size_t)o.c; c0 += per) {
            const size_t nc = std::min(per, (size_t)o.c - c0);
            FFGPU_CHECK(hipMemcpy2D(g_bounce, row, src + c0 * plane * ex->N, row * ex->N, row, nc, hipMemcpyDeviceToHost));
            memcpy(host_out + c0 * plane, g_bounce, nc * row);
        }
    }
    return (int)(plane * o.c);
}

static int timed_issue(ffgpu_exec *ex, const float *d_frames, int reps, std::vector<float> &us)
{
    hipStream_t s = ex->own_stream;
    const InputSrc in = fp32_src(d_frames);
    if (push_params(ex, in, s)) return -1;
    const size_t n = ex->steps.size();
    std::vector<hipEvent_t> ev(n + 1, nullptr);
    us.assign(n, 0.f);
    auto run = [&]() -> int {
        for (auto &e : ev) FFGPU_CHECK(hipEventCreate(&e));
        if (issue_all(ex, in, s)) return -1;
        for (int r = 0; r < reps; r++) {
            FFGPU_CHECK(hipEventRecord(ev[0], s));
            for (size_t i = 0; i < n; i++) {
                if (issue_step(ex, ex->steps[i], in, s)) return -1;
                FFGPU_CHECK(hipEventRecord(ev[i + 1], s));
            }
            FFGPU_CHECK(hipStreamSynchronize(s));
            for (size_t i = 0; i < n; i++) {
                float ms = 0.f;
                FFGPU_CHECK(hipEventElapsedTime(&ms, ev[i], ev[i + 1]));
                us[i] += ms * 1000.f / reps;
            }
// ... 124 lines not shown

extern "C" int ffgpu_netdev_profile_us(void *p, double us_by_kind[LAYER_TYPE_TOTOAL])
{
    ffgpu_netdev *dev = (ffgpu_netdev *)p;
    if (!dev) return -1;
    for (int k = 0; k < LAYER_TYPE_TOTOAL; k++) us_by_kind[k] = dev->us_acc[k];
    return 0;
}

extern "C" int ffgpu_net_weights_dev(NET *net, void **dev_ptr, size_t *bytes)
{
    ffgpu_netdev *dev = netdev_of(net);
    if (!dev) return -1;
    if (dev_ptr) *dev_ptr = dev->d_weights;
    if (bytes) *bytes = sizeof(float) * (size_t)net->weight_size;
    return 0;
}

extern "C" int ffgpu_net_weights_commit(NET *net, void *stream)
{
    ffgpu_netdev *dev = netdev_of(net);
    if (!dev) return -1;
    std::lock_guard<std::mutex> lk(dev->mu);
    for (ffgpu_exec *ex : dev->execs)
        if (repack(ex, stream ? (hipStream_t)stream : ex->own_stream)) return -1;
    if (!stream) for (ffgpu_exec *ex : dev->execs) FFGPU_CHECK(hipStreamSynchronize(ex->own_stream));
    return 0;
}

#include "ffgpu_node.inc"

static void fill_desc(ConvDesc &d, const float *in, const float *filt, float *out, int batch,
                      int iw, int ih, int ic, int groups, int pad, int stride, int fs, int ow, int oh, int oc, int act, int flags)
{
    memset(&d, 0, sizeof d);
    d.in = in; d.filt = filt; d.out = out; d.N = batch;
    d.iw = iw; d.ih = ih; d.ic = ic; d.ow = ow; d.oh = oh; d.oc = oc;
    d.fs = fs; d.stride = stride; d.pad = pad; d.groups = groups; d.act = act; d.flags = flags & (FFGPU_COMPAT_V6 | FFGPU_BF16_PW);
    d.in_cs = (long)batch * iw * ih; d.in_ns = (long)iw * ih;
    d.out_cs = (long)batch * ow * oh; d.out_ns = (long)ow * oh;
}

extern "C" int ffgpu_groupconv_dev(const float *d_in, const float *d_filt, float *d_out, int batch,
                                   int iw, int ih, int ic, int groups, int pad, int stride,
                                   int fs, int fn, int ow, int oh, int oc, int act,
                                   int flags, int variant, void *stream)
{
    if (!d_in || !d_filt || !d_out || batch < 1 || fn != oc) { ffgpu_set_error("groupconv_dev: bad arguments"); return -1; }
    ConvDesc d;
    fill_desc(d, d_in, d_filt, d_out, batch, iw, ih, ic, groups, pad, stride, fs, ow, oh, oc, act, flags);
    return ffgpu_launch_conv(d, variant, (hipStream_t)stream);
}

extern "C" const char *ffgpu_groupconv_kernel_name(int batch, int iw, int ih, int ic, int groups, int pad,
                                                   int stride, int fs, int fn, int variant)
{
    ConvDesc d;
    const int ow = (iw + 2 * pad - fs) / stride + 1, oh = (ih + 2 * pad - fs) / stride + 1;
    fill_desc(d, nullptr, nullptr, nullptr, batch, iw, ih, ic, groups, pad, stride, fs, ow, oh, fn, 0, 0);
    return ffgpu_conv_kernel_name(d, variant);
}

extern "C" float ffgpu_groupconv_time_dev(const float *d_in, const float *d_filt, float *d_out, int batch,
                                          int iw, int ih, int ic, int groups, int pad, int stride,
                                          int fs, int fn, int ow, int oh, int oc, int act,
                                          int flags, int variant, int warmup, int iters, void *stream)
{
    if (iters < 1 || fn != oc) { ffgpu_set_error("groupconv_time_dev: bad arguments"); return -1.f; }
    hipStream_t s = (hipStream_t)stream;
    ConvDesc d;
    fill_desc(d, d_in, d_filt, d_out, batch, iw, ih, ic, groups, pad, stride, fs, ow, oh, oc, act, flags);
    float *pk = nullptr;
    if (variant == FFGPU_K_AUTO && ffgpu_pw_pack_floats(d) > 0) {
        if (hipMalloc(&pk, ffgpu_pw_pack_floats(d) * sizeof(float)) != hipSuccess || ffgpu_pw_pack(d, pk, s)) { ffgpu_set_error("pack failed"); return -1.f; }
        d.wpack = pk;
    }
    hipEvent_t e0, e1;
    if (hipEventCreate(&e0) != hipSuccess || hipEventCreate(&e1) != hipSuccess) { ffgpu_set_error("hipEventCreate failed"); return -1.f; }
    for (int i = 0; i < warmup; i++) if (ffgpu_launch_conv(d, variant, s)) return -1.f;
    (void)hipEventRecord(e0, s);
    for (int i = 0; i < iters; i++) if (ffgpu_launch_conv(d, variant, s)) return -1.f;
    (void)hipEventRecord(e1, s);
    if (hipEventSynchronize(e1) != hipSuccess) { ffgpu_set_error("hipEventSynchronize: %s", hipGetErrorString(hipGetLastError())); return -1.f; }
    float ms = 0.f;
    (void)hipEventElapsedTime(&ms, e0, e1);
    (void)hipEventDestroy(e0); (void)hipEventDestroy(e1);
    return ms * 1000.f / iters;
}

static void irb_fill(IrbDesc &d, int batch, int iw, int ih, int ic, int ec, int oc, int stride, int act1, int actd, int act2, int res_act)
{
    d.N = batch; d.H = ih; d.W = iw; d.OH = (ih + 2 - 3) / stride + 1; d.OW = (iw + 2 - 3) / stride + 1;
    d.ic = ic; d.ec = ec; d.oc = oc; d.stride = stride;
    d.act1 = act1; d.actd = actd; d.act2 = act2; d.res_act = res_act;
}

extern "C" int ffgpu_irb_plan_text(int batch, int iw, int ih, int ic, int ec, int oc, int stride, int act1, int actd, int act2, int res_act, int flags, char *buf, int cap)
{
    if (!buf || cap < 1 || batch < 1 || iw < 1 || ih < 1 || stride < 1) { ffgpu_set_error("irb_plan_text: bad arguments"); return -1; }
    IrbDesc d{};
    irb_fill(d, batch, iw, ih, ic, ec, oc, stride, act1, actd, act2, res_act);
    d.flags = flags & FFGPU_CONCURRENT;
    (void)ffgpu_irb_plan(d);
    return ffgpu_irb_plan_line(d, buf, (size_t)cap);
}

// ... 162 lines not shown
```

### ffcnn_amd/csrc/ffgpu_kernels.hip

```cpp
#include <algorithm>
#include <type_traits>
#include <vector>
#include <mutex>
#include <cstdio>
#include <cstdlib>
#include <cstring>
#include "ffgpu_dev.hpp"
#include "ffgpu_knobs.hpp"

#define WAVE 64

#define FFG __attribute__((address_space(1)))
typedef const FFG float *gfp;
__device__ __forceinline__ gfp to_global(const float *p) { return (gfp)p; }
template <class T> __device__ __forceinline__ T gld(gfp p) { return *(const FFG T *)p; }

__device__ __forceinline__ float act_apply(float x, int act)
{
    switch (act) {
    case 1: return x > 0.f ? x : 0.f;
    case 2: return x > 0.f ? x : 0.1f * x;
    case 3: return 1.0f / (1.0f + (float)exp((double)-x));
    default: return x;
    }
// ... 132 lines not shown
}

__global__ void k_upsample(const float *in, float *out, long planes, int w, int h, int stride)
{
    const int ow = w * stride, oh = h * stride;
    const long total = planes * oh * ow;
    for (long idx = (long)blockIdx.x * blockDim.x + threadIdx.x; idx < total; idx += (long)gridDim.x * blockDim.x) {
        const int x = (int)(idx % ow);
        const long t = idx / ow;
        const int y = (int)(t % oh);
        out[idx] = in[((t / oh) * h + y / stride) * w + x / stride];
    }
}

__global__ void __launch_bounds__(256) k_upsample32(const float *in, float *out, unsigned n_in, int w, int h, int stride, unsigned m_w, unsigned m_h)
{
    const int ow = w * stride;
    for (unsigned idx = blockIdx.x * blockDim.x + threadIdx.x; idx < n_in; idx += gridDim.x * blockDim.x) {
        const unsigned t = m_w ? __umulhi(idx, m_w) : idx;
        const unsigned x = idx - t * w;
        const unsigned pl = m_h ? __umulhi(t, m_h) : t;
        const unsigned y = t - pl * h;
        const float v = in[idx];
        float *o = out + ((size_t)pl * h * stride + y * stride) * ow + x * stride;
        for (int dy = 0; dy < stride; dy++)
            for (int dx = 0; dx < stride; dx++) o[dy * ow + dx] = v;
    }
}

__global__ void k_add_act(const float *a, const float *b, float *out, long n, int act)
{
    const long n4 = n >> 2;
    const long gid = (long)blockIdx.x * blockDim.x + threadIdx.x, gsz = (long)gridDim.x * blockDim.x;
    for (long i = gid; i < n4; i += gsz) {
        const float4 u = reinterpret_cast<const float4 *>(a)[i], v = reinterpret_cast<const float4 *>(b)[i];
        float4 r;
        r.x = act_apply(u.x + v.x, act); r.y = act_apply(u.y + v.y, act);
        r.z = act_apply(u.z + v.z, act); r.w = act_apply(u.w + v.w, act);
        reinterpret_cast<float4 *>(out)[i] = r;
    }
    for (long i = (n4 << 2) + gid; i < n; i += gsz) out[i] = act_apply(a[i] + b[i], act);
}

__global__ void k_copy(const float *src, float *dst, long n)
{
    const long n4 = n >> 2;
    const long gid = (long)blockIdx.x * blockDim.x + threadIdx.x, gsz = (long)gridDim.x * blockDim.x;
    for (long i = gid; i < n4; i += gsz) reinterpret_cast<float4 *>(dst)[i] = reinterpret_cast<const float4 *>(src)[i];
    for (long i = (n4 << 2) + gid; i < n; i += gsz) dst[i] = src[i];
}

#include "ffgpu_block.inc"

__global__ void k_yolo(YoloHead hd, int N, int netw, int neth, BBOX *cand, int *cand_key, int *ncand, int cap, int *ring_ctr)
{
#pragma clang fp contract(off)
    if (ring_ctr && blockIdx.x == 0 && threadIdx.x == 0) *ring_ctr += 1;
    const int cells = hd.w * hd.h;
    const long total = (long)N * 3 * cells;
    const long gid = (long)blockIdx.x * blockDim.x + threadIdx.x;
    const int lane = threadIdx.x & 63;
    const long gidc = min(gid, total - 1);
    const int cell = (int)(gidc % cells);
    const int k = (int)((gidc / cells) % 3);
    const int n = (int)(gidc / (3L * cells));
    const int j = cell % hd.w, i = cell / hd.w;
    const long cs = (long)N * cells;
    const float *p = hd.in + (long)k * (5 + hd.classes) * cs + (long)n * cells + cell;
    const float bs = p[4 * cs];
    const bool pass = gid < total && !(1.0f / (1.0f + __expf(-bs)) < hd.thresh * 0.999f);
    float cs_best = 0.f;
    int best = 0;
    for (unsigned long long todo = __ballot(pass); todo; todo &= todo - 1) {
        const int src = __ffsll((long long)todo) - 1;
        const long g = gid - lane + src;
        const int c2 = (int)(g % cells), k2 = (int)((g / cells) % 3), n2 = (int)(g / (3L * cells));
        const float *q = hd.in + (long)k2 * (5 + hd.classes) * cs + (long)n2 * cells + c2;
        float v = -INFINITY;
        int vi = 1 << 30;
        for (int l = lane ? lane : 64; l < hd.classes; l += 64) {
            const float t = q[(5 + l) * cs];
            if (v < t) { v = t; vi = l; }
        }
#pragma unroll
        for (int off = 32; off > 0; off >>= 1) {
            const float ov = __shfl_xor(v, off);
            const int oi = __shfl_xor(vi, off);
            if (v < ov || (v == ov && oi < vi)) { v = ov; vi = oi; }
        }
        const float c0 = q[5 * cs];
        if (lane == src) { const bool up = c0 < v; cs_best = up ? v : c0; best = up ? vi : 0; }
    }
    if (!pass) return;
    const float conf = 1.0f / ((1.0f + (float)exp((double)-bs) * (1.0f + (float)exp((double)-cs_best))));
    if (!(conf >= hd.thresh)) return;
    const float tx = p[0], ty = p[cs], tw = p[2 * cs], th = p[3 * cs];
    const float sx = 1.0f / (1.0f + (float)exp((double)-tx));
    const float sy = 1.0f / (1.0f + (float)exp((double)-ty));
    const float cx = (j + sx) * netw / hd.w;
    const float cy = (i + sy) * neth / hd.h;
    const float bw = (float)exp((double)tw) * hd.anchors[k][0] * hd.scale_xy;
    const float bh = (float)exp((double)th) * hd.anchors[k][1] * hd.scale_xy;
    const int slot = atomicAdd(&ncand[n], 1);
    if (slot >= cap) return;
    BBOX b;
    b.type = best; b.score = conf;
    b.x1 = cx - bw * 0.5f; b.y1 = cy - bh * 0.5f;
    b.x2 = cx + bw * 0.5f; b.y2 = cy + bh * 0.5f;
    cand[(long)n * cap + slot] = b;
    cand_key[(long)n * cap + slot] = hd.key_base + cell * 3 + k;
}

template <bool GLB>
__global__ void __launch_bounds__(256) k_nms(const BBOX *cand, const int *cand_key, int *ncand, int cap, int cap_p2,
                                             BBOX *full, unsigned char *scratch,
                                             ffgpu_frame_dets *dets, ffgpu_frame_dets *dets_host,
                                             const int *ring_ctr, float thresh, int use_min, const ExecParams *prm)
{
#pragma clang fp contract(off)
    extern __shared__ __attribute__((aligned(16))) unsigned char nms_lds[];
    unsigned char *wb = GLB ? scratch + (size_t)blockIdx.x * cap_p2 * 13 : nms_lds;
    float *s_score = reinterpret_cast<float *>(wb);
    int   *s_key = reinterpret_cast<int *>(wb + (size_t)4 * cap_p2);
// ... 151 lines not shown
    const size_t lds = (size_t)4 * w * h * sizeof(float);
    if (lds_allow((const void *)k_spp, lds, "spp")) return -1;
    hipLaunchKernelGGL(k_spp, dim3((unsigned)std::min((planes + 1) / 2, 4096L)), dim3(256), lds, s, p);
    LAUNCH_OK("spp");
    return 0;
}

int ffgpu_launch_upsample(const float *in, float *out, long planes, int w, int h, int stride, hipStream_t s)
{
    const long total = planes * h * stride * w * stride, n_in = planes * h * w;
    if (n_in * std::max(w, h) < (1L << 32) && total < (1L << 32)) {
        auto magic = [](long dv) { return dv == 1 ? 0u : (unsigned)(((1ULL << 32) + (unsigned long long)dv - 1) / (unsigned long long)dv); };
        hipLaunchKernelGGL(k_upsample32, dim3(grid_for(n_in, 256)), dim3(256), 0, s, in, out, (unsigned)n_in, w, h, stride, magic(w), magic(h));
        LAUNCH_OK("upsample");
        return 0;
    }
    hipLaunchKernelGGL(k_upsample, dim3(grid_for(total, 256)), dim3(256), 0, s, in, out, planes, w, h, stride);
    LAUNCH_OK("upsample");
    return 0;
}

int ffgpu_launch_add_act(const float *a, const float *b, float *out, long n, int act, hipStream_t s)
{
    hipLaunchKernelGGL(k_add_act, dim3(grid_for((n + 3) / 4, 256)), dim3(256), 0, s, a, b, out, n, act);
    LAUNCH_OK("add_act");
    return 0;
}

__global__ void k_hash64(const unsigned *x, long n, unsigned long long *out)
{
    unsigned long long h = 0;
    for (long i = (long)blockIdx.x * blockDim.x + threadIdx.x; i < n; i += (long)gridDim.x * blockDim.x) {
        unsigned long long v = ((unsigned long long)x[i] << 32 | (unsigned long long)(unsigned)i) + 0x9e3779b97f4a7c15ull * (unsigned long long)(i >> 32);
        v ^= v >> 30; v *= 0xbf58476d1ce4e5b9ull; v ^= v >> 27; v *= 0x94d049bb133111ebull; v ^= v >> 31;
        h += v;
    }
    for (int o = 32; o > 0; o >>= 1) h += __shfl_xor(h, o);
    if ((threadIdx.x & 63) == 0) atomicAdd(out, h);
}
int ffgpu_launch_hash64(const float *x, long n, unsigned long long *out, hipStream_t s)
{
    hipLaunchKernelGGL(k_hash64, dim3(grid_for(n, 256, 256 * 16)), dim3(256), 0, s, reinterpret_cast<const unsigned *>(x), n, out);
    LAUNCH_OK("hash64");
    return 0;
}

int ffgpu_launch_copy(const float *src, float *dst, long n, hipStream_t s)
{
    hipLaunchKernelGGL(k_copy, dim3(grid_for((n + 3) / 4, 256)), dim3(256), 0, s, src, dst, n);
    LAUNCH_OK("copy");
    return 0;
}

int ffgpu_launch_yolo(const YoloHead &hd, int N, int netw, int neth, BBOX *cand, int *cand_key, int *ncand, int cap, int *ring_ctr, hipStream_t s)
{
    const long total = (long)N * 3 * hd.w * hd.h;
    hipLaunchKernelGGL(k_yolo, dim3((unsigned)((total + 255) / 256)), dim3(256), 0, s, hd, N, netw, neth, cand, cand_key, ncand, cap, ring_ctr);
    LAUNCH_OK("yolo");
    return 0;
}

bool ffgpu_nms_in_lds(int cap_pow2)
{
    if (cap_pow2 > FFGPU_NMS_LDS_CAP) return false;
    int dev = 0, lds = 0;
    (void)hipGetDevice(&dev);
    if (hipDeviceGetAttribute(&lds, hipDeviceAttributeMaxSharedMemoryPerBlock, dev) != hipSuccess || lds <= 0) { (void)hipGetLastError(); lds = 64 * 1024; }
    return (size_t)13 * cap_pow2 <= (size_t)lds;
}

int ffgpu_launch_nms(const BBOX *cand, const int *cand_key, int *ncand, int cap, BBOX *full, void *scratch,
                     ffgpu_frame_dets *dets, ffgpu_frame_dets *dets_host, const int *ring_ctr, int N,
                     float thresh, int use_min, const ExecParams *prm, hipStream_t s)
{
    int p2 = 1;
    while (p2 < cap) p2 <<= 1;
    if (!ffgpu_nms_in_lds(p2)) {
        if (!scratch) { ffgpu_set_error("nms: %d candidate slots per frame need the global scratch buffer", cap); return -1; }
        hipLaunchKernelGGL(k_nms<true>, dim3(N), dim3(256), 0, s, cand, cand_key, ncand, cap, p2, full, (unsigned char *)scratch,
                           dets, dets_host, ring_ctr, thresh, use_min, prm);
    } else {
        const size_t lds = (size_t)13 * p2;
        if (lds_allow((const void *)k_nms<false>, lds > 64 * 1024 ? (size_t)13 * FFGPU_NMS_LDS_CAP : lds, "nms")) return -1;
        hipLaunchKernelGGL(k_nms<false>, dim3(N), dim3(256), lds, s, cand, cand_key, ncand, cap, p2, full, nullptr,
                           dets, dets_host, ring_ctr, thresh, use_min, prm);
    }
    LAUNCH_OK("nms");
    return 0;
}

int ffgpu_launch_set_params(ExecParams *d_prm, const ExecParams &v, hipStream_t s)
{
    hipLaunchKernelGGL(k_set_params, dim3(1), dim3(1), 0, s, d_prm, v);
    LAUNCH_OK("set_params");
    return 0;
}

int ffgpu_launch_clear(int *ncand, int N, int *ring_ctr, hipStream_t s)
{
    hipLaunchKernelGGL(k_clear, dim3((N + 255) / 256), dim3(256), 0, s, ncand, N, ring_ctr);
    LAUNCH_OK("clear");
    return 0;
}

__global__ void __launch_bounds__(256) k_pack_records(const ffgpu_frame_dets *recs, long slot_stride_recs, int batch, int cap, unsigned char *out, long out_stride)
{
    __shared__ int s_first[1025];
    const ffgpu_frame_dets *r = recs + (long)blockIdx.x * slot_stride_recs;
    unsigned char *o = out + (long)blockIdx.x * out_stride;
    int *hdr = reinterpret_cast<int *>(o);
// ... 50 lines not shown
```

### ffcnn_amd/csrc/ffgpu_knobs.hpp

```cpp
#pragma once
#include <assert.h>
#include <limits.h>
#include <stdio.h>
#include <stdlib.h>

enum KnobKind { KNOB_INT, KNOB_ON, KNOB_SET, KNOB_TEXT };
enum KnobClass { KNOB_PRODUCT, KNOB_TUNING, KNOB_TEST, KNOB_LAB };
#define KNOB_COMPUTED INT_MIN

#define FFGPU_KNOBS_MAIN(X) \
     \
    X(COMPAT_V6,         "FFCNN_COMPAT_V6",         ON,   0,             PRODUCT, "the reference's v6 behaviour for 5x5 filters (executors and groupconv)") \
    X(NO_GRAPH,          "FFGPU_NO_GRAPH",          ON,   0,             PRODUCT, "eager launches instead of a captured graph (as the flag FFGPU_NO_GRAPH)") \
    X(BF16_PW,           "FFGPU_BF16_PW",           ON,   0,             PRODUCT, "opt-in bf16 inputs for compute-bound pointwise layers; own tolerance (as the flag)") \
    X(NO_FUSE,           "FFGPU_NO_FUSE",           ON,   0,             PRODUCT, "one kernel per layer: no fused blocks, no concat in place, no residual in the conv epilogue (as the flag)") \
    X(BRANCH,            "FFGPU_BRANCH",            ON,   0,             PRODUCT, "first detection head as a parallel graph branch instead of in line") \
    X(DWPW,              "FFGPU_DWPW",              ON,   0,             PRODUCT, "the heads' depthwise + pointwise pairs as one kernel (measured slower)") \
    X(NO_U8_FRONT,       "FFGPU_NO_U8_FRONT",       SET,  0,             PRODUCT, "u8 frames through the staging kernel and the fp32 first kernel even where they could go straight in") \
    X(NV12_FRONT,        "FFGPU_NV12_FRONT",        INT,  KNOB_COMPUTED, PRODUCT, "1: NV12 frames into the NV12 form of k_front where the plan has it, 0: staged; default: the build's measured choice") \
    X(VERBOSE,           "FFGPU_VERBOSE",           SET,  0,             PRODUCT, "print every error to stderr as it is set") \
    X(NODE_PACK_BOXES,   "FFGPU_NODE_PACK_BOXES",   INT,  0,             PRODUCT, "room per frame in a shard's packed record block; 0 or less: 16, the constant of the same name in ffgpu_node.inc") \
    X(NO_IRB,            "FFGPU_NO_IRB",            ON,   0,             TUNING,  "no fused inverted-residual blocks: their three layers as three kernels") \
    X(IRB_MIN_EC,        "FFGPU_IRB_MIN_EC",        INT,  24,            TUNING,  "fewest expanded channels of a block the planner fuses (thin blocks apart)") \
    X(IRB_STAGE,         "FFGPU_IRB_STAGE",         INT,  1,             TUNING,  "runs of 48 -> 224 -> 48 blocks on a small plane as one launch in FFGPU_CONCURRENT executors of 32 frames or more (0: one launch per block)") \
// ... 4 lines not shown
    X(PW_X3,             "FFGPU_PW_X3",             INT,  1,             PRODUCT, "0: never pick the split-bf16 pointwise kernel k_pw_x3") \
    X(PWX3_MIN_IC,       "FFGPU_PWX3_MIN_IC",       INT,  192,           TUNING,  "k_pw_x3: fewest input channels AUTO takes it for") \
    X(PWX3_MIN_OC,       "FFGPU_PWX3_MIN_OC",       INT,  256,           TUNING,  "k_pw_x3: fewest output channels") \
    X(PWX3_MIN_P,        "FFGPU_PWX3_MIN_P",        INT,  65536,         TUNING,  "k_pw_x3: fewest pixels") \
    X(PWX3_MT,           "FFGPU_PWX3_MT",           INT,  0,             TUNING,  "k_pw_x3: 16-row blocks per wave, 1 / 2 / 4 (0: 4)") \
    X(PW_X3T,            "FFGPU_PW_X3T",            INT,  1,             PRODUCT, "0: never pick the tiled split-bf16 GEMM k_pw_x3t") \
    X(PWX3T_MIN_IC,      "FFGPU_PWX3T_MIN_IC",      INT,  128,           TUNING,  "k_pw_x3t: fewest input channels AUTO takes it for") \
    X(PWX3T_MIN_OC,      "FFGPU_PWX3T_MIN_OC",      INT,  192,           TUNING,  "k_pw_x3t: fewest output channels") \
    X(PWX3T_MIN_P,       "FFGPU_PWX3T_MIN_P",       INT,  65536,         TUNING,  "k_pw_x3t: fewest pixels") \
    X(PWXT_TM,           "FFGPU_PWXT_TM",           INT,  256,           TUNING,  "k_pw_x3t: channels per workgroup tile, 256 or 128 (frozen with a plan: ConvDesc::x3_mt)") \
    X(PWXT_NARROW,       "FFGPU_PWXT_NARROW",       INT,  1,             TUNING,  "k_pw_x3t: 0 switches the narrow tiles of the partial last round off") \
    X(PWXT_PERSIST,      "FFGPU_PWXT_PERSIST",      INT,  0,             TUNING,  "k_pw_x3t: persistent workgroups over the main tiles") \
    X(PWXT_NT,           "FFGPU_PWXT_NT",           INT,  -1,            TUNING,  "k_pw_x3t: non-temporal output stores never (0) / always (1); -1: outputs of 128 MB and more") \
    X(PWXT_DBG,          "FFGPU_PWXT_DBG",          INT,  0,             LAB,     "k_pw_x3t: ablation mask handed to the kernel (wrong results)") \
    X(PW_X3S,            "FFGPU_PW_X3S",            INT,  1,             PRODUCT, "0: never pick the pointwise form of k_conv_x3 (pw_x3s)") \
    X(PWX3S_MIN_IC,      "FFGPU_PWX3S_MIN_IC",      INT,  96,            TUNING,  "pw_x3s: fewest input channels AUTO takes it for") \
    X(PWX3S_MIN_OC,      "FFGPU_PWX3S_MIN_OC",      INT,  64,            TUNING,  "pw_x3s: fewest output channels") \
    X(PWX3S_MIN_WGS,     "FFGPU_PWX3S_MIN_WGS",     INT,  64,            TUNING,  "pw_x3s: fewest workgroups") \
    X(IG_X3,             "FFGPU_IG_X3",             INT,  1,             PRODUCT, "0: never pick the split-bf16 dense 3x3 kernel k_conv_x3") \
    X(IGX3_S2,           "FFGPU_IGX3_S2",           INT,  1,             TUNING,  "k_conv_x3: 0 keeps the stride-2 layers on the fp32 implicit GEMM") \
    X(IGX3_NW,           "FFGPU_IGX3_NW",           INT,  0,             TUNING,  "k_conv_x3: waves per workgroup, 4 or 8 (0: 8 at stride 2, else 4)") \
    X(IGX3_MT,           "FFGPU_IGX3_MT",           INT,  0,             TUNING,  "k_conv_x3: 16-row blocks per wave, 1 / 2 / 4 (0: by shape; frozen with a plan: ConvDesc::x3_mt)") \
    X(IGX3_MT4_WGS,      "FFGPU_IGX3_MT4_WGS",      INT,  192,           TUNING,  "k_conv_x3: fewest workgroups that four blocks per wave must leave") \
    X(IGX3_MIN_IC,       "FFGPU_IGX3_MIN_IC",       INT,  16,            TUNING,  "k_conv_x3: fewest input channels AUTO takes it for") \
    X(IGX3_MIN_WGS,      "FFGPU_IGX3_MIN_WGS",      INT,  160,           TUNING,  "k_conv_x3: fewest workgroups AUTO takes it for") \
    X(PWG_MIN_OC,        "FFGPU_PWG_MIN_OC",        INT,  128,           TUNING,  "k_pw_gemm32: fewest output channels AUTO takes it for") \
    X(PWG_MIN_IC,        "FFGPU_PWG_MIN_IC",        INT,  64,            TUNING,  "k_pw_gemm32: fewest input channels") \
    X(NO_PW_GEMM,        "FFGPU_NO_PW_GEMM",        INT,  0,             PRODUCT, "never pick k_pw_gemm32: k_pw_mfma instead") \
    X(NO_IGEMM,          "FFGPU_NO_IGEMM",          INT,  0,             TUNING,  "never pick the implicit GEMMs (k_conv_igemm, the dense form of k_conv_x3)") \
    X(NO_GROUP_THIN,     "FFGPU_NO_GROUP_THIN",     INT,  0,             TUNING,  "never pick k_conv_thin for grouped layers of few channels per group") \
    X(NO_DW_PAIR,        "FFGPU_NO_DW_PAIR",        INT,  0,             PRODUCT, "depthwise layers on k_dw_lds instead of k_dw_pair") \
    X(NO_CONV_FIRST,     "FFGPU_NO_CONV_FIRST",     INT,  0,             PRODUCT, "the first layer on the dense small-channel kernel instead of k_conv_first") \
    X(CONV_FIRST_MIN_PX, "FFGPU_CONV_FIRST_MIN_PX", INT,  262144,        TUNING,  "k_conv_first: fewest output pixels of the batch") \
    X(NO_POOL2X2,        "FFGPU_NO_POOL2X2",        INT,  0,             TEST,    "2x2 / stride 2 max pooling on the general pool kernel") \
     \
    X(IGEMM_NOVEC,       "FFGPU_IGEMM_NOVEC",       INT,  0,             TUNING,  "k_conv_igemm: no vector form of the gather") \
    X(IGEMM_SPLIT,       "FFGPU_IGEMM_SPLIT",       INT,  0,             TUNING,  "k_conv_igemm: split-K factor 1 .. 16 (0: by tile count; frozen with a plan: ConvDesc::nsplit)") \
    X(DW_U,              "FFGPU_DW_U",              INT,  4,             TUNING,  "k_dw3_stream: rows per step, 1 / 2 / 4") \
    X(DW_BAND,           "FFGPU_DW_BAND",           INT,  4,             TUNING,  "k_dw3_stream: rows per wave task (0: enough tasks to fill the chip)") \
    X(DW_NT,             "FFGPU_DW_NT",             INT,  -1,            PRODUCT, "k_dw3_stream: stream past the caches never (0) / always (1); -1: outputs of 128 MB and more") \
    X(DW_XCD,            "FFGPU_DW_XCD",            INT,  0,             TUNING,  "k_dw3_stream: walk the tasks XCD by XCD") \
    X(DWP_NI,            "FFGPU_DWP_NI",            INT,  0,             TUNING,  "k_dw_pair: frames per workgroup, at most (0: by shape)") \
    X(DWL_BH,            "FFGPU_DWL_BH",            INT,  0,             TUNING,  "k_dw_lds: rows per band (0: by shape)") \
    X(DWL_NPL,           "FFGPU_DWL_NPL",           INT,  0,             TUNING,  "k_dw_lds: planes per item (0: by shape)") \
    X(PWG_WM,            "FFGPU_PWG_WM",            INT,  0,             TUNING,  "k_pw_gemm32: waves per workgroup, 4 or 8 (0: 8 from 248 output channels; part of the packed image)") \
    X(PWG_NARROW,        "FFGPU_PWG_NARROW",        INT,  1,             TUNING,  "k_pw_gemm32: 0 switches the narrow tiles of the partial last round off") \
    X(PWG_DBG,           "FFGPU_PWG_DBG",           INT,  0,             LAB,     "k_pw_gemm32: ablation mask handed to the kernel (wrong results)") \
     \
    X(NO_THIN,           "FFGPU_NO_THIN",           INT,  0,             PRODUCT, "8-channel blocks on the wave kernel instead of k_irb_thin") \
    X(THIN_BAND,         "FFGPU_THIN_BAND",         INT,  KNOB_COMPUTED, TUNING,  "k_irb_thin: rows per wave; default by batch and height (thin_band)") \
    X(THIN_PAIR,         "FFGPU_THIN_PAIR",         INT,  1,             TUNING,  "k_irb_thin: 0 keeps FFGPU_CONCURRENT executors off the paired form (two frames per wave, 3 / 4 / 5 columns per lane); read at launch") \
    X(THIN_S2,           "FFGPU_THIN_S2",           INT,  1,             TUNING,  "k_irb_thin_s2: 0 keeps FFGPU_CONCURRENT executors off the streaming form of the stride-2 block 4 -> 24 -> 8 (the planned wave kernel instead); read at launch") \
    X(THIN_S2_BAND,      "FFGPU_THIN_S2_BAND",      INT,  0,             TUNING,  "k_irb_thin_s2: output rows per wave (0: by batch and height, thin_s2_form); read at launch") \
    X(FRONT_BAND,        "FFGPU_FRONT_BAND",       INT,  KNOB_COMPUTED, TUNING,  "k_front: rows per wave; default as FFGPU_THIN_BAND") \
    X(NO_FRONT,          "FFGPU_NO_FRONT",          INT,  0,             PRODUCT, "layers 0-3 as k_conv_first + k_irb_thin instead of k_front") \
    X(FRONT_MIN_PX,      "FFGPU_FRONT_MIN_PX",      INT,  262144,        TUNING,  "k_front: fewest output pixels of the batch") \
    X(FRONT_NC,          "FFGPU_FRONT_NC",          INT,  3,             PRODUCT, "k_front: output columns per lane, 3 where a row fits a wave that way, or 4") \
    X(NO_IRBW,           "FFGPU_NO_IRBW",           INT,  0,             PRODUCT, "fused blocks on the workgroup kernel k_irb instead of the wave-autonomous k_irbw") \
    X(IRBW_S2_633,       "FFGPU_IRBW_S2_633",       INT,  1,             TUNING,  "k_irbw: 0 hides the stride-2 form for 24 input / 48 output channels from the planner") \
    X(IRBW_S2_NSI4,      "FFGPU_IRBW_S2_NSI4",      INT,  0,             TUNING,  "k_irbw: 1 lets the planner take the four-strip halo for the thin stride-2 blocks") \
    X(IRBW_TWQ,          "FFGPU_IRBW_TWQ",          INT,  0,             TUNING,  "k_irbw: tile width in quads (with FFGPU_IRBW_TH; 0: searched)") \
    X(IRBW_TH,           "FFGPU_IRBW_TH",           INT,  0,             TUNING,  "k_irbw: tile height (with FFGPU_IRBW_TWQ; 0: searched)") \
    X(IRBW_BIG,          "FFGPU_IRBW_BIG",          INT,  -1,            TUNING,  "k_irbw: the 256-register form never (0) / always (1); -1: by register need") \
    X(IRBW_BIG_S2K1,     "FFGPU_IRBW_BIG_S2K1",     INT,  -1,            TUNING,  "k_irbw: as FFGPU_IRBW_BIG for the stride-2 blocks of at most 4 input channels alone") \
    X(IRBW_GWAVES,       "FFGPU_IRBW_GWAVES",       INT,  KNOB_COMPUTED, TUNING,  "k_irbw: waves a launch wants before the group split stops; default 1200, 500 with FFGPU_CONCURRENT") \
    X(IRBW_NOEXC,        "FFGPU_IRBW_NOEXC",        INT,  0,             TUNING,  "k_irbw: without the measured exception (four waves on the 20x20 blocks)") \
    X(IRBW_G_MID,        "FFGPU_IRBW_G_MID",        INT,  0,             TUNING,  "k_irbw: group split for 256 .. 1099 tiles (0: as computed)") \
    X(IRBW_X3,           "FFGPU_IRBW_X3",           INT,  30,            PRODUCT, "fused blocks: expand GEMM as split-bf16 products, one bit per shape: 0: 8 input channels, 1: 16, 2: 24, 3: 48 (split tile in LDS), 4: the 40 -> 20 stride-2 block") \
    X(IRBW_G_XL,         "FFGPU_IRBW_G_XL",         INT,  7,             TUNING,  "k_irbw: group split of the LDS-resident form with several chains in flight") \
    X(IRBW_G_SMALL,      "FFGPU_IRBW_G_SMALL",      INT,  0,             TUNING,  "k_irbw: group split under 256 tiles (0: as computed)") \
    X(IRBW_G,            "FFGPU_IRBW_G",            INT,  0,             TUNING,  "k_irbw: group split, wins over everything (0: as computed)") \
    X(IRBW_NSO,          "FFGPU_IRBW_NSO",          INT,  2,             TUNING,  "k_irbw2: anything but 2 keeps the planner off the two-strip kernel") \
    X(IRBW2_TWQ,         "FFGPU_IRBW2_TWQ",         INT,  0,             TUNING,  "k_irbw2: tile width in quads (with FFGPU_IRBW2_TH; 0: searched)") \
    X(IRBW2_TH,          "FFGPU_IRBW2_TH",          INT,  0,             TUNING,  "k_irbw2: tile height (with FFGPU_IRBW2_TWQ; 0: searched)") \
    X(IRBW2_MIN_TILES,   "FFGPU_IRBW2_MIN_TILES",   INT,  768,           TUNING,  "k_irbw2: fewest tiles the planner takes it for") \
    X(IRBW_WPB,          "FFGPU_IRBW_WPB",          INT,  0,             TUNING,  "k_irbw: tiles per workgroup without a group split, 1 .. 8 (0: 4 or 8 by LDS)") \
    X(IRBW_HALF,         "FFGPU_IRBW_HALF",         INT,  1,             PRODUCT, "0: a last group of at most 8 real expanded channels is computed as a whole group") \
    X(IRBW_XCD,          "FFGPU_IRBW_XCD",          INT,  3,             PRODUCT, "fused blocks walk their tiles XCD by XCD; bit 0: one-wave-per-tile launches, bit 1: group-split launches") \
    X(IRBW_FOLD,         "FFGPU_IRBW_FOLD",         INT,  0,             TUNING,  "k_irbw: never widen the reduction region to all G partial sums (folding rounds)") \
    X(IRB_ECH,           "FFGPU_IRB_ECH",           INT,  0,             TUNING,  "k_irb: expanded channels per chunk, 16 or 32 (0: by shape)") \
    X(IRB_RESIDENT,      "FFGPU_IRB_RESIDENT",      INT,  1,             TUNING,  "k_irb: every chunk's constants in LDS never (0) / where it costs no workgroup (1) / wherever they fit (2)") \
    X(IRB_TW,            "FFGPU_IRB_TW",            INT,  0,             TUNING,  "k_irb: tile width (0: the measured table, then the search)") \
    X(IRB_TH,            "FFGPU_IRB_TH",            INT,  0,             TUNING,  "k_irb: tile height for the search (0: any)") \
    X(IRB_NF,            "FFGPU_IRB_NF",            INT,  0,             TUNING,  "k_irb: frames per tile for the search, 1 / 2 / 4 (0: any)") \
    X(IRB_NOTABLE,       "FFGPU_IRB_NOTABLE",       INT,  0,             TUNING,  "k_irb: skip the measured table of tiles, search") \
    X(IRB_NW,            "FFGPU_IRB_NW",            INT,  8,             TUNING,  "k_irb: waves per workgroup, 8 or 4") \
    X(IRB_NOKS,          "FFGPU_IRB_NOKS",          INT,  0,             TUNING,  "k_irb: idle waves take no slices of the channel loop") \
    X(IRB_SKIP,          "FFGPU_IRB_SKIP",          INT,  0,             LAB,     "k_irb: ablation mask, 1 no input loads, 2 no expand, 4 no depthwise / project, 8 no stores (wrong results)") \
    X(IRB_TRACE,         "FFGPU_IRB_TRACE",         INT,  0,             LAB,     "lab builds with -DIRB_TRACE=1: every fused-block launch is followed by its in-kernel timeline on stderr") \
    X(VERBOSE_IRB,       "FFGPU_VERBOSE_IRB",       INT,  0,             LAB,     "print the plan line of every fused-block launch to stderr")

#ifdef FFGPU_DIAG
#define FFGPU_KNOBS_DIAG(X) \
    X(DBG_SKIP,          "FFGPU_DBG_SKIP",          TEXT, 0,             LAB,     "make DIAG=1: \"lo:hi\" drops the launches of layers lo .. hi (wrong results)") \
    X(DBG_KEEP,          "FFGPU_DBG_KEEP",          TEXT, 0,             LAB,     "make DIAG=1: \"lo:hi\" drops every launch but those of layers lo .. hi (wrong results)")
#else
#define FFGPU_KNOBS_DIAG(X)
#endif
#if defined(XT_TRACE) && XT_TRACE
#define FFGPU_KNOBS_XT(X) \
    X(PWXT_TRACE,        "FFGPU_PWXT_TRACE",        TEXT, 0,             LAB,     "builds with -DXT_TRACE=1: file that one traced k_pw_x3t launch dumps its per-tile timeline to")
#else
#define FFGPU_KNOBS_XT(X)
#endif
#define FFGPU_KNOBS(X) FFGPU_KNOBS_MAIN(X) FFGPU_KNOBS_DIAG(X) FFGPU_KNOBS_XT(X)

// ... 46 lines not shown
```

### include/ffcnn_hip.h

```cpp
#ifndef FFCNN_AMD_FFCNN_HIP_H
#define FFCNN_AMD_FFCNN_HIP_H

#include <stddef.h>
#include "ffcnn.h"

#ifdef __cplusplus
extern "C" {
#endif

#define FFGPU_MAX_DET   128



typedef struct {
    int  count;
    int  ncand;
    int  overflow;
    int  nfull;
    BBOX box[FFGPU_MAX_DET];
} ffgpu_frame_dets;

typedef struct ffgpu_exec ffgpu_exec;

#define FFGPU_KEEP_ALL   1
// ... 90 lines not shown
int         ffgpu_node_depth(const ffgpu_node *node);
int         ffgpu_node_rccl_ranks(const ffgpu_node *node);
float      *ffgpu_node_input_dev(ffgpu_node *node, int rank);
float      *ffgpu_node_input_slot_dev(ffgpu_node *node, int rank, int slot);
int         ffgpu_node_forward(ffgpu_node *node, ffgpu_frame_dets *host_out);
int         ffgpu_node_forward_host(ffgpu_node *node, const float *h_frames, ffgpu_frame_dets *host_out);
long        ffgpu_node_submit(ffgpu_node *node, const float *h_frames);
int         ffgpu_node_wait(ffgpu_node *node, long ticket, ffgpu_frame_dets *host_out);
int         ffgpu_node_run(ffgpu_node *node, long steps, ffgpu_frame_dets *host_out);

int ffgpu_groupconv_dev(const float *d_in, const float *d_filt, float *d_out, int batch,
                        int iw, int ih, int ic, int groups, int pad, int stride,
                        int fs, int fn, int ow, int oh, int oc, int act,
                        int flags, int variant, void *stream);

enum {
    FFGPU_K_AUTO = 0,
    FFGPU_K_GENERIC = 1,
    FFGPU_K_DW_STREAM = 2,
    FFGPU_K_DW_LDS = 3,
    FFGPU_K_PW_MFMA = 4,
    FFGPU_K_PW_GEMM = 5,
    FFGPU_K_DENSE_SMALL = 7,
    FFGPU_K_IGEMM = 8,
    FFGPU_K_PW_BF16 = 9,
    FFGPU_K_GROUP_THIN = 10,
    FFGPU_K_PW_X3 = 11,
    FFGPU_K_CONV_X3 = 12,
    FFGPU_K_PW_X3T = 13
};

const char *ffgpu_groupconv_kernel_name(int batch, int iw, int ih, int ic, int groups, int pad,
                                        int stride, int fs, int fn, int variant);

float ffgpu_groupconv_time_dev(const float *d_in, const float *d_filt, float *d_out, int batch,
                               int iw, int ih, int ic, int groups, int pad, int stride,
                               int fs, int fn, int ow, int oh, int oc, int act,
                               int flags, int variant, int warmup, int iters, void *stream);

float ffgpu_irb_dev(const float *d_in, const float *d_w1, const float *d_wd, const float *d_w2,
                    const float *d_res, float *d_out, int batch, int iw, int ih, int ic, int ec, int oc,
                    int stride, int act1, int actd, int act2, int res_act, int warmup, int iters, void *stream);

float ffgpu_irb_flags_dev(const float *d_in, const float *d_w1, const float *d_wd, const float *d_w2,
                          const float *d_res, float *d_out, int batch, int iw, int ih, int ic, int ec, int oc,
                          int stride, int act1, int actd, int act2, int res_act, int flags, int warmup, int iters, void *stream);

int ffgpu_irb_thin_launch_text(int batch, int iw, int ih, int ic, int ec, int oc, int stride, int act1, int actd, int act2, int res_act,
                               int flags, char *buf, int cap);

int ffgpu_irb_s2_launch_text(int batch, int iw, int ih, int ic, int ec, int oc, int stride, int act1, int actd, int act2, int res_act,
                             int flags, char *buf, int cap);

int ffgpu_irb_plan_text(int batch, int iw, int ih, int ic, int ec, int oc, int stride, int act1, int actd, int act2, int res_act,
                        int flags, char *buf, int cap);

int ffgpu_irb_stage_plan_text(int batch, int iw, int ih, int blocks, int act1, int actd, int flags, char *buf, int cap);

int ffgpu_front_plan_text(int batch, int pw, int ph, int form, char *buf, int cap);

int ffgpu_irb_instantiations(char *buf, int cap);

int ffgpu_knobs_text(char *buf, int cap);

float ffgpu_dwpw_dev(const float *d_in, const float *d_wd, const float *d_wp, float *d_out, int batch, int iw, int ih,
                     int c, int oc, int fs, int actd, int actp, int warmup, int iters, void *stream);

size_t ffgpu_packed_records_bytes(int batch, int cap);
int    ffgpu_unpack_records(const void *block, int batch, int cap, ffgpu_frame_dets *out);
int    ffgpu_pack_records(const void *d_records, int nslots, long slot_stride_records, int batch, int cap, void *d_out, void *stream);

typedef struct {
    int image;
    int x0, y0;
    int reserved;
} ffgpu_tile;

#define FFGPU_MERGE_LDS_SLOTS 1024

size_t ffgpu_merge_tiles_scratch_bytes(int ntiles, int list_stride);
int    ffgpu_merge_tiles_dev(const void *d_records, const void *d_lists, int list_stride, const ffgpu_tile *tiles, int ntiles, int nimages,
                             float thresh, int use_min, void *d_out_records, void *d_out_lists, void *d_scratch, size_t scratch_bytes, void *stream);

int ffgpu_exec_merge_tiles(ffgpu_exec *ex, const ffgpu_tile *tiles, int ntiles, int nimages, void *stream);
int ffgpu_exec_merged_dev(ffgpu_exec *ex, void **dev_ptr, size_t *bytes);
int ffgpu_exec_read_merged(ffgpu_exec *ex, ffgpu_frame_dets *host_out, int max_images);
int ffgpu_exec_read_merged_boxes(ffgpu_exec *ex, int image, BBOX *host_out, int cap);

typedef struct { int x0, y0, w, h; } ffgpu_tile_rect;
int ffgpu_tile_plan(int img_w, int img_h, int tile_w, int tile_h, int overlap_x, int overlap_y, int align, ffgpu_tile_rect *out, int cap);

typedef struct {
    unsigned char color[4];
    const unsigned char *palette;
    int npalette;
    int thickness;
} ffgpu_draw_style;

int ffgpu_draw_boxes_bgr_dev (const void *d_records, const void *d_lists, int list_stride, const int *list_first,
                              const ffgpu_bgr_frame  *targets, int ntargets, const ffgpu_draw_style *style, void *stream);
int ffgpu_draw_boxes_nv12_dev(const void *d_records, const void *d_lists, int list_stride, const int *list_first,
                              const ffgpu_nv12_frame *targets, int ntargets, const ffgpu_draw_style *style, void *stream);

#define FFGPU_DRAW_ENTRIES 0
#define FFGPU_DRAW_MERGED  1
int ffgpu_exec_draw_bgr (ffgpu_exec *ex, int which, const ffgpu_bgr_frame  *targets, int ntargets, const ffgpu_draw_style *style, void *stream);
// ... 532 lines not shown
```

Before: 209,900.

## Split YOLO head conv into box pass and sparse class pass over passing quads

The pointwise conv feeding each YOLO head is split in two. A box pass computes the 15 box/objectness rows for every pixel and appends the quads whose objectness can pass the threshold to a list via a ballot plus atomicAdd. A class pass then computes the class rows only for listed quads, skipping most of the class-channel work, with a fallback to all quads when the list overflows. This adds an extra launch and a counter reset in k_yolo. Class outputs for skipped pixels are left unwritten, which relies on the decode only reading them for passing cells.

Result: faster. 215,900, median of 6 (+2.9%).

```diff
diff --git a/ffcnn_amd/capi.py b/ffcnn_amd/capi.py
--- a/ffcnn_amd/capi.py
+++ b/ffcnn_amd/capi.py
@@ -302,7 +302,7 @@
            "ffgpu_exec_kernel_count", "ffgpu_exec_work_model", "ffgpu_exec_set_scale", "ffgpu_exec_forward_dev", "ffgpu_exec_forward_host",
            "ffgpu_exec_forward_bgr_dev", "ffgpu_exec_forward_bgr_frames_dev", "ffgpu_exec_forward_nv12_frames_dev", "ffgpu_exec_dets_dev", "ffgpu_exec_dets_host", "ffgpu_exec_set_ring", "ffgpu_exec_set_ring_strided", "ffgpu_exec_read_dets", "ffgpu_exec_read_layer", "ffgpu_exec_hash_layers",
            "ffgpu_exec_read_boxes", "ffgpu_exec_cand_capacity", "ffgpu_exec_graph_captures",
-           "ffgpu_exec_profile", "ffgpu_exec_profile_steps", "ffgpu_exec_step_model", "ffgpu_groupconv_dev", "ffgpu_groupconv_kernel_name", "ffgpu_groupconv_time_dev", "ffgpu_irb_dev", "ffgpu_irb_flags_dev", "ffgpu_irb_plan_text", "ffgpu_irb_thin_launch_text", "ffgpu_irb_s2_launch_text", "ffgpu_irb_stage_plan_text", "ffgpu_front_plan_text", "ffgpu_irb_instantiations", "ffgpu_knobs_text", "ffgpu_dwpw_dev", "ffgpu_packed_records_bytes", "ffgpu_pack_records", "ffgpu_unpack_records",
+           "ffgpu_exec_profile", "ffgpu_exec_profile_steps", "ffgpu_exec_step_model", "ffgpu_groupconv_dev", "ffgpu_groupconv_kernel_name", "ffgpu_groupconv_time_dev", "ffgpu_irb_dev", "ffgpu_irb_flags_dev", "ffgpu_irb_plan_text", "ffgpu_irb_thin_launch_text", "ffgpu_irb_s2_launch_text", "ffgpu_sparse_head_dev", "ffgpu_sparse_head_launch_text", "ffgpu_irb_stage_plan_text", "ffgpu_front_plan_text", "ffgpu_irb_instantiations", "ffgpu_knobs_text", "ffgpu_dwpw_dev", "ffgpu_packed_records_bytes", "ffgpu_pack_records", "ffgpu_unpack_records",
            "ffgpu_shard_range", "ffgpu_node_create", "ffgpu_node_destroy", "ffgpu_node_ndev", "ffgpu_node_shard", "ffgpu_node_set_scale",
            "ffgpu_node_input_dev", "ffgpu_node_input_slot_dev", "ffgpu_node_depth", "ffgpu_node_rccl_ranks", "ffgpu_node_forward", "ffgpu_node_forward_host",
            "ffgpu_node_submit", "ffgpu_node_wait", "ffgpu_node_run",
@@ -407,6 +407,8 @@
     L.ffgpu_irb_flags_dev.argtypes = [vp] * 6 + [i] * 14 + [vp]
     L.ffgpu_irb_thin_launch_text.argtypes = [i] * 12 + [C.c_char_p, i]
     L.ffgpu_irb_s2_launch_text.argtypes = [i] * 12 + [C.c_char_p, i]
+    L.ffgpu_sparse_head_dev.argtypes = [vp, vp, vp] + [i] * 6 + [C.c_float, vp, vp, vp]
+    L.ffgpu_sparse_head_launch_text.argtypes = [i] * 6 + [C.c_char_p, i]
     L.ffgpu_irb_plan_text.argtypes = [i] * 12 + [C.c_char_p, i]
     L.ffgpu_irb_stage_plan_text.argtypes = [i] * 7 + [C.c_char_p, i]
     L.ffgpu_front_plan_text.argtypes = [i] * 4 + [C.c_char_p, i]
@@ -1752,6 +1754,17 @@
     return buf.value.decode()
 
 
+def sparse_head_dev(d_in, d_filt, d_out, batch, iw, ih, ic, classes, thresh, d_list, d_count, act=0, stream=None):
+    _check(lib().ffgpu_sparse_head_dev(d_in, d_filt, d_out, batch, iw, ih, ic, classes, act, thresh, d_list, d_count, stream), "ffgpu_sparse_head_dev")
+
+
+def sparse_head_launch_text(batch, iw, ih, ic, classes, flags=0):
+    buf = C.create_string_buffer(256)
+    if lib().ffgpu_sparse_head_launch_text(batch, iw, ih, ic, classes, flags, buf, len(buf)) < 0:
+        raise RuntimeError("ffgpu_sparse_head_launch_text failed: %s" % last_error())
+    return buf.value.decode()
+
+
 def irb_dev(d_in, d_w1, d_wd, d_w2, d_res, d_out, batch, iw, ih, ic, ec, oc, stride, act1=2, actd=2, act2=0, res_act=0,
             warmup=0, iters=0, stream=None, flags=0):
     us = lib().ffgpu_irb_flags_dev(d_in, d_w1, d_wd, d_w2, d_res, d_out, batch, iw, ih, ic, ec, oc, stride, act1, actd, act2, res_act, flags,
diff --git a/ffcnn_amd/csrc/ffgpu_conv_kernels.inc b/ffcnn_amd/csrc/ffgpu_conv_kernels.inc
--- a/ffcnn_amd/csrc/ffgpu_conv_kernels.inc
+++ b/ffcnn_amd/csrc/ffgpu_conv_kernels.inc
@@ -250,7 +250,16 @@
 }
 static int ig_x3_mt(const ConvDesc &d) { const int m = d.x3_mt == 4 || d.x3_mt == 2 || d.x3_mt == 1 ? d.x3_mt : ig_x3_mt_plan(d); return d.stride == 2 && m > 2 ? 2 : m; }
 static void ig_x3_dims(const ConvDesc &d, int &MT, int &ngr, int &nrb, int &ntm) { MT = ig_x3_mt(d); ngr = (d.fs * (d.ic / 8) + 3) / 4; nrb = (d.oc + 15) / 16; ntm = (nrb + MT - 1) / MT; }
-static size_t ig_x3_img_dwords(const ConvDesc &d) { int MT, ngr, nrb, ntm; ig_x3_dims(d, MT, ngr, nrb, ntm); return (size_t)ntm * ngr * 3 * d.fs * MT * 256; }
+static bool ig_x3_sparse(const ConvDesc &d) { return d.sp_classes > 0 && d.fs == 1 && d.oc == 3 * (5 + d.sp_classes); }
+static void ig_x3_sp_dims(const ConvDesc &d, int sp, int &MT, int &ngr, int &nrb, int &ntm)
+{
+    ig_x3_dims(d, MT, ngr, nrb, ntm);
+    if (sp == 1) { MT = 1; nrb = 1; }
+    if (sp == 2) nrb = (3 * d.sp_classes + 15) / 16;
+    ntm = (nrb + MT - 1) / MT;
+}
+static size_t ig_x3_sp_dwords(const ConvDesc &d, int sp) { int MT, ngr, nrb, ntm; ig_x3_sp_dims(d, sp, MT, ngr, nrb, ntm); return (size_t)ntm * ngr * 3 * d.fs * MT * 256; }
+static size_t ig_x3_img_dwords(const ConvDesc &d) { return ig_x3_sp_dwords(d, 0) + (ig_x3_sparse(d) ? ig_x3_sp_dwords(d, 1) + ig_x3_sp_dwords(d, 2) : 0); }
 static bool ig_x3_auto(const ConvDesc &d)
 {
     if (!ig_x3_ok(d)) return false;
@@ -263,14 +272,18 @@
 }
 static int ig_x3_pack(const ConvDesc &d, float *pk, hipStream_t s)
 {
-    IgX3PackP q;
-    int nrb;
-    q.filt = d.filt; q.pk = reinterpret_cast<unsigned *>(pk); q.ic = d.ic; q.oc = d.oc; q.k4 = conv_k4(d); q.fs = d.fs;
-    ig_x3_dims(d, q.MT, q.ngr, nrb, q.ntm);
-    q.nunits = d.fs * (d.ic / 8);
-    const long total = (long)ig_x3_img_dwords(d);
-    hipLaunchKernelGGL(k_conv_x3_pack, dim3((unsigned)std::min((total + 255) / 256, 8192L)), dim3(256), 0, s, q);
-    LAUNCH_OK("conv_x3_pack");
+    unsigned *img = reinterpret_cast<unsigned *>(pk);
+    for (int sp = 0; sp <= (ig_x3_sparse(d) ? 2 : 0); sp++) {
+        IgX3PackP q;
+        int nrb;
+        q.filt = d.filt; q.pk = img; q.ic = d.ic; q.oc = d.oc; q.k4 = conv_k4(d); q.fs = d.fs; q.sp = sp; q.classes = d.sp_classes;
+        ig_x3_sp_dims(d, sp, q.MT, q.ngr, nrb, q.ntm);
+        q.nunits = d.fs * (d.ic / 8);
+        const long total = (long)ig_x3_sp_dwords(d, sp);
+        hipLaunchKernelGGL(k_conv_x3_pack, dim3((unsigned)std::min((total + 255) / 256, 8192L)), dim3(256), 0, s, q);
+        LAUNCH_OK("conv_x3_pack");
+        img += total;
+    }
     return 0;
 }
 
@@ -616,16 +629,18 @@
     return 0;
 }
 
-static int launch_conv_x3(const ConvDesc &d, const float *image, hipStream_t s)
+static int launch_conv_x3_form(const ConvDesc &d, const float *image, int sp, hipStream_t s)
 {
     IgX3P p;
     int MT;
     p.in = d.in; p.out = d.out; p.residual = d.residual; p.filt = d.filt;
     p.iw = d.iw; p.ih = d.ih; p.ow = d.ow; p.oh = d.oh; p.ic = d.ic; p.oc = d.oc; p.k4 = conv_k4(d); p.act = d.act; p.res_act = d.res_act;
     p.in_cs = (unsigned)d.in_cs; p.in_ns = (unsigned)d.in_ns;
-    ig_x3_dims(d, MT, p.ngr, p.nrb, p.ntm);
+    ig_x3_sp_dims(d, sp, MT, p.ngr, p.nrb, p.ntm);
     p.nunits = d.fs * (d.ic / 8);
-    p.wpack = reinterpret_cast<const unsigned *>(image);
+    p.wpack = reinterpret_cast<const unsigned *>(image) + (sp >= 1 ? ig_x3_sp_dwords(d, 0) : 0) + (sp == 2 ? ig_x3_sp_dwords(d, 1) : 0);
+    p.sp_list = d.sp_list; p.sp_ctr = d.sp_ctr; p.sp_classes = d.sp_classes; p.sp_thresh = d.sp_thresh;
+    p.sp_cap = (int)((long)d.N * d.oh * d.ow / 4);
     const int NW = ig_x3_nw(d);
     p.owp = d.fs == 1 ? d.ow : (d.ow + 3) & ~3; p.P = (long)d.N * d.oh * d.ow; p.Pp = (long)d.N * d.oh * p.owp;
     p.ntn = (p.Pp + 63) / 64; p.npg = (p.ntn + NW - 1) / NW;
@@ -633,6 +648,15 @@
     if (nblk > (1L << 30)) { ffgpu_set_error("conv_x3: too many tiles"); return -1; }
     const size_t lds = (size_t)2 * 3 * d.fs * MT * 1024 + (size_t)MT * 128;
     const dim3 grid((unsigned)nblk);
+    if (sp) {
+#define IGX3_LAUNCH_SP(mt, nw, spv) do { if (lds_allow((const void *)k_conv_x3<mt, nw, 1, 1, spv>, lds, "conv_x3")) return -1; hipLaunchKernelGGL((k_conv_x3<mt, nw, 1, 1, spv>), grid, dim3(64 * nw), lds, s, p); } while (0)
+        if (sp == 1) { if (NW == 8) IGX3_LAUNCH_SP(1, 8, 1); else IGX3_LAUNCH_SP(1, 4, 1); }
+        else if (NW == 8) { if (MT == 4) IGX3_LAUNCH_SP(4, 8, 2); else if (MT == 2) IGX3_LAUNCH_SP(2, 8, 2); else IGX3_LAUNCH_SP(1, 8, 2); }
+        else              { if (MT == 4) IGX3_LAUNCH_SP(4, 4, 2); else if (MT == 2) IGX3_LAUNCH_SP(2, 4, 2); else IGX3_LAUNCH_SP(1, 4, 2); }
+#undef IGX3_LAUNCH_SP
+        LAUNCH_OK(sp == 1 ? "conv_x3 (box pass)" : "conv_x3 (class pass)");
+        return 0;
+    }
 #define IGX3_LAUNCH(mt, nw, fs) do { if (lds_allow((const void *)k_conv_x3<mt, nw, fs>, lds, "conv_x3")) return -1; hipLaunchKernelGGL((k_conv_x3<mt, nw, fs>), grid, dim3(64 * nw), lds, s, p); } while (0)
 #define IGX3_LAUNCH2(mt, nw) do { if (d.fs == 1) IGX3_LAUNCH(mt, nw, 1); else IGX3_LAUNCH(mt, nw, 3); } while (0)
     if (d.stride == 2) {
@@ -647,6 +671,31 @@
 #undef IGX3_LAUNCH
     LAUNCH_OK("conv_x3");
     return 0;
+}
+
+static int launch_conv_x3(const ConvDesc &d, const float *image, hipStream_t s)
+{
+    if (!(ig_x3_sparse(d) && d.sp_list && d.sp_ctr && !d.residual)) return launch_conv_x3_form(d, image, 0, s);
+    return launch_conv_x3_form(d, image, 1, s) || launch_conv_x3_form(d, image, 2, s) ? -1 : 0;
+}
+
+int ffgpu_conv_sparse_head_line(const ConvDesc &d0, int classes, bool wanted, char *buf, size_t cap)
+{
+    ConvDesc d = d0;
+    ffgpu_conv_plan(d);
+    if (!wanted || !ffgpu_conv_sparse_head_ok(d, classes)) return snprintf(buf, cap, "dense %s", ffgpu_conv_kernel_name(d, FFGPU_K_AUTO));
+    d.sp_classes = classes;
+    int MT, ngr, nrb, ntm1, ntm2;
+    ig_x3_sp_dims(d, 1, MT, ngr, nrb, ntm1);
+    ig_x3_sp_dims(d, 2, MT, ngr, nrb, ntm2);
+    const long slots = (ig_x3_npg(d) + 7) / 8 * 8;
+    return snprintf(buf, cap, "sparse box<1,%d> rows=15 grid=%ld class<%d,%d> rows=%d grid=%ld quads=%ld image=%zu", ig_x3_nw(d), slots * ntm1, MT, ig_x3_nw(d),
+                    3 * classes, slots * ntm2, (long)d.N * d.oh * d.ow / 4, ig_x3_img_dwords(d));
+}
+
+bool ffgpu_conv_sparse_head_ok(const ConvDesc &d, int classes)
+{
+    return classes >= 1 && d.fs == 1 && d.oc == 3 * (5 + classes) && !d.residual && conv_pick(d, FFGPU_K_AUTO) == FFGPU_K_CONV_X3 && ig_x3_ok(d);
 }
 
 static int launch_igemm(const ConvDesc &d, const float *image, hipStream_t s)
diff --git a/ffcnn_amd/csrc/ffgpu_conv_x3.inc b/ffcnn_amd/csrc/ffgpu_conv_x3.inc
--- a/ffcnn_amd/csrc/ffgpu_conv_x3.inc
+++ b/ffcnn_amd/csrc/ffgpu_conv_x3.inc
@@ -8,9 +8,20 @@
     int  nunits, ngr;
     int  nrb, ntm;
     int  act, res_act;
+    int *sp_list, *sp_ctr;
+    int  sp_cap, sp_classes;
+    float sp_thresh;
 };
 
-struct IgX3PackP { const float *filt; unsigned *pk; int ic, oc, k4, nunits, ngr, ntm, MT, fs; };
+template <int SP>
+__host__ __device__ static inline int x3_sp_chan(int classes, int r)
+{
+    if (SP == 1) return r < 15 ? (r / 5) * (5 + classes) + r % 5 : -1;
+    if (SP == 2) return r < 3 * classes ? (r / classes) * (5 + classes) + 5 + r % classes : -1;
+    return r;
+}
+
+struct IgX3PackP { const float *filt; unsigned *pk; int ic, oc, k4, nunits, ngr, ntm, MT, fs, sp, classes; };
 __global__ void k_conv_x3_pack(IgX3PackP p)
 {
     const int nkx = p.fs;
@@ -24,16 +35,18 @@
         const int kx = (int)(t % nkx); t /= nkx;
         const int gr = (int)(t % p.ngr), mt = (int)(t / p.ngr);
         const int u = 4 * gr + (l >> 4), cb8 = u / nkx, ky = u - nkx * cb8;
-        const int o = 16 * (mt * p.MT + rb) + (l & 15), c = u < p.nunits ? 8 * cb8 + 2 * d : p.ic;
-        const float w0 = (o < p.oc && c < p.ic) ? p.filt[(long)o * rl + (c * nkx + ky) * nkx + kx] : 0.f;
-        const float w1 = (o < p.oc && c + 1 < p.ic) ? p.filt[(long)o * rl + ((c + 1) * nkx + ky) * nkx + kx] : 0.f;
+        const int r = 16 * (mt * p.MT + rb) + (l & 15), c = u < p.nunits ? 8 * cb8 + 2 * d : p.ic;
+        const int o = p.sp == 1 ? x3_sp_chan<1>(p.classes, r) : (p.sp == 2 ? x3_sp_chan<2>(p.classes, r) : r);
+        const float w0 = (o >= 0 && o < p.oc && c < p.ic) ? p.filt[(long)o * rl + (c * nkx + ky) * nkx + kx] : 0.f;
+        const float w1 = (o >= 0 && o < p.oc && c + 1 < p.ic) ? p.filt[(long)o * rl + ((c + 1) * nkx + ky) * nkx + kx] : 0.f;
         p.pk[i] = irbw_x3_part(w0, part) | (irbw_x3_part(w1, part) << 16);
     }
 }
 
-template <int MT, int NW, int FS, int ST = 1>
+template <int MT, int NW, int FS, int ST = 1, int SP = 0>
 __global__ void __launch_bounds__(64 * NW, 8 / NW) __attribute__((amdgpu_waves_per_eu(2))) k_conv_x3(IgX3P p)
 {
+    static_assert(SP == 0 || (FS == 1 && ST == 1), "the sparse forms are pointwise");
     constexpr int NKX = FS, NCOL = FS == 1 ? 4 : (ST == 2 ? 9 : 6);
     constexpr int CH = 3 * NKX * MT * 256;
     typedef v4f_x3 v4a4 __attribute__((aligned(4)));
@@ -47,19 +60,32 @@
     const int mtile = (int)(rr_ % p.ntm);
     const long pg = (rr_ / p.ntm) * 8 + xcd;
     if (pg >= p.npg) return;
+    unsigned sp_cnt = 0; bool sp_all = false;
+    if (SP == 2) {
+        const unsigned c = (unsigned)*p.sp_ctr;
+        sp_all = c > (unsigned)p.sp_cap;
+        sp_cnt = sp_all ? (unsigned)p.sp_cap : c;
+        if ((unsigned long)pg * (16 * NW) >= sp_cnt) return;
+    }
     const int rb0 = mtile * MT;
     float *sb = reinterpret_cast<float *>(igx_lds + 2 * CH);
     {
         const int rl = p.k4 + 4;
         for (int i = tid; i < MT * 32; i += 64 * NW) {
-            const int o = 16 * rb0 + (i >> 1);
-            sb[i] = o < p.oc ? p.filt[(long)o * rl + p.k4 + (i & 1)] : 0.f;
+            const int o = x3_sp_chan<SP>(p.sp_classes, 16 * rb0 + (i >> 1));
+            sb[i] = (o >= 0 && o < p.oc) ? p.filt[(long)o * rl + p.k4 + (i & 1)] : 0.f;
         }
     }
 
     const long pxt = pg * NW + wid;
-    const long pq = pxt * 64 + 4 * n;
-    const bool qvalid = pq < p.Pp;
+    long pq = pxt * 64 + 4 * n;
+    bool qvalid = pq < p.Pp;
+    if (SP == 2) {
+        const unsigned slot = (unsigned)pxt * 16u + (unsigned)n;
+        qvalid = slot < sp_cnt;
+        const unsigned quad = !qvalid ? 0u : (sp_all ? slot : min((unsigned)p.sp_list[slot], (unsigned)p.sp_cap - 1u));
+        pq = 4L * quad;
+    }
     const unsigned pqu = (unsigned)(qvalid ? pq : 0);
     unsigned qn = 0; int qy = 0, qa = 0, qskip = 0;
     unsigned base_pix = pqu;
@@ -229,6 +255,7 @@
     }
 
     if (!qvalid) return;
+    bool sp_hit = false;
     const float slope = p.act == 2 ? 0.1f : (p.act == 1 ? 0.f : 1.f), rslope = p.res_act == 2 ? 0.1f : (p.res_act == 1 ? 0.f : 1.f);
     const long px = FS == 3 ? ((long)qn * p.oh + qy) * p.ow + qa : pq;
     const bool vec = FS == 1 || (p.owp == p.ow && (p.P & 3) == 0);
@@ -236,8 +263,8 @@
     for (int t = 0; t < MT; t++)
 #pragma unroll
         for (int r = 0; r < 4; r++) {
-            const int o = 16 * (rb0 + t) + 4 * kq + r;
-            if (o < p.oc) {
+            const int o = x3_sp_chan<SP>(p.sp_classes, 16 * (rb0 + t) + 4 * kq + r);
+            if (o >= 0 && o < p.oc) {
                 const float sc = sb[2 * (16 * t + 4 * kq + r)], bi = sb[2 * (16 * t + 4 * kq + r) + 1];
                 v4f_pw v = pw_fma4_apart(acc[t][0][r], acc[t][1][r], acc[t][2][r], acc[t][3][r], sc, bi);
                 v = pw_act4(v, slope, p.act == 3);
@@ -258,6 +285,19 @@
 #pragma unroll
                     for (int q = 0; q < 4; q++) if (q >= qskip) p.out[off + q] = v[q];
                 }
+                if (SP == 1 && (4 * kq + r) % 5 == 4)
+                    sp_hit = sp_hit || yolo_obj_pass(v[0], p.sp_thresh) || yolo_obj_pass(v[1], p.sp_thresh) || yolo_obj_pass(v[2], p.sp_thresh) || yolo_obj_pass(v[3], p.sp_thresh);
             }
         }
+    if (SP == 1) {
+        const unsigned long long hit = __ballot(sp_hit);
+        const unsigned m16 = (unsigned)((hit | (hit >> 16) | (hit >> 32) | (hit >> 48)) & 0xffffu);
+        if (m16) {
+            int base = 0;
+            if (lane == 0) base = atomicAdd(p.sp_ctr, __popc(m16));
+            base = __builtin_amdgcn_readfirstlane(base);
+            const int slot = base + __popc(m16 & ((1u << n) - 1u));
+            if (kq == 0 && ((m16 >> n) & 1u) && (unsigned)slot < (unsigned)p.sp_cap) p.sp_list[slot] = (int)(pq >> 2);
+        }
+    }
 }
diff --git a/ffcnn_amd/csrc/ffgpu_dev.hpp b/ffcnn_amd/csrc/ffgpu_dev.hpp
--- a/ffcnn_amd/csrc/ffgpu_dev.hpp
+++ b/ffcnn_amd/csrc/ffgpu_dev.hpp
@@ -43,6 +43,9 @@
     int   nsplit;
     int   kernel;
     int   x3_mt;
+    int   sp_classes;
+    float sp_thresh;
+    int  *sp_list, *sp_ctr;
 };
 #define FFGPU_F_BATCH_INPUT (1 << 30)
 
@@ -136,7 +139,9 @@
     float thresh, scale_xy;
     int   key_base;
 };
-int ffgpu_launch_yolo(const YoloHead &hd, int N, int netw, int neth, BBOX *cand, int *cand_key, int *ncand, int cap, int *ring_ctr, hipStream_t s);
+int ffgpu_launch_yolo(const YoloHead &hd, int N, int netw, int neth, BBOX *cand, int *cand_key, int *ncand, int cap, int *ring_ctr, int *sp_ctr, hipStream_t s);
+bool ffgpu_conv_sparse_head_ok(const ConvDesc &d, int classes);
+int  ffgpu_conv_sparse_head_line(const ConvDesc &d, int classes, bool wanted, char *buf, size_t cap);
 int ffgpu_launch_nms(const BBOX *cand, const int *cand_key, int *ncand, int cap, BBOX *full, void *scratch,
                      ffgpu_frame_dets *dets, ffgpu_frame_dets *dets_host, const int *ring_ctr, int N,
                      float thresh, int use_min, const ExecParams *prm, hipStream_t s);
diff --git a/ffcnn_amd/csrc/ffgpu_exec.hip b/ffcnn_amd/csrc/ffgpu_exec.hip
--- a/ffcnn_amd/csrc/ffgpu_exec.hip
+++ b/ffcnn_amd/csrc/ffgpu_exec.hip
@@ -143,6 +143,7 @@
     float   *out2[2];
     int      fs2[2];
     int      lane;
+    int     *sp_ctr;
 };
 
 struct ffgpu_netdev {
@@ -190,6 +191,7 @@
     float *arena = nullptr;
     float *d_input = nullptr;
     float *d_pack = nullptr;
+    int   *d_sparse = nullptr;
     BBOX  *d_cand = nullptr;
     int   *d_cand_key = nullptr, *d_ncand = nullptr;
     int    cand_cap = 1, bbox_max = 1;
@@ -457,6 +459,40 @@
     }
 }
 
+static bool sparse_head_wanted(int flags) { return (flags & FFGPU_CONCURRENT) && !(flags & (FFGPU_KEEP_ALL | FFGPU_NO_FUSE)) && knob(K_SPARSE_HEAD) != 0; }
+
+static void sparse_heads(ffgpu_exec *ex)
+{
+    if (!sparse_head_wanted(ex->flags)) return;
+    std::vector<Step> &S = ex->steps;
+    for (Step &y : S) {
+        if (y.kind != S_YOLO) continue;
+        for (Step &c : S) {
+            if (c.kind != S_CONV || c.layer < 0 || c.layer != y.layer - 1 || ex->layout.canon[c.layer] != c.layer || ex->layout.nuses[c.layer] != 1 ||
+                c.in_is_input || c.conv.out != y.head.in) continue;
+            if (!ffgpu_conv_sparse_head_ok(c.conv, y.head.classes)) continue;
+            c.conv.sp_classes = y.head.classes; c.conv.sp_thresh = y.head.thresh;
+            ex->layout.readable[c.layer] = 0;
+        }
+    }
+}
+
+static int place_sparse(ffgpu_exec *ex)
+{
+    size_t tot = 0;
+    for (const Step &st : ex->steps) if (st.kind == S_CONV && st.conv.sp_classes) tot += 64 + (size_t)st.conv.N * st.conv.oh * st.conv.ow / 4;
+    if (!tot) return 0;
+    if (hipMalloc(&ex->d_sparse, tot * sizeof(int)) != hipSuccess || hipMemsetAsync(ex->d_sparse, 0, tot * sizeof(int), ex->own_stream) != hipSuccess) { ffgpu_set_error("hipMalloc(sparse heads) failed"); return -1; }
+    size_t off = 0;
+    for (Step &st : ex->steps) {
+        if (st.kind != S_CONV || !st.conv.sp_classes) continue;
+        st.conv.sp_ctr = ex->d_sparse + off; st.conv.sp_list = ex->d_sparse + off + 64;
+        for (Step &y : ex->steps) if (y.kind == S_YOLO && y.layer - 1 == st.layer) y.sp_ctr = st.conv.sp_ctr;
+        off += 64 + (size_t)st.conv.N * st.conv.oh * st.conv.ow / 4;
+    }
+    return 0;
+}
+
 static void rewrite_steps(ffgpu_exec *ex)
 {
     std::vector<Step> &S = ex->steps;
@@ -468,6 +504,7 @@
         S.erase(std::remove_if(S.begin(), S.end(), [](const Step &t) { return t.kind == S_CLEAR; }), S.end());
     }
     { Step nm{}; nm.kind = S_NMS; nm.layer = -1; nm.ltype = LAYER_TYPE_YOLO; S.push_back(nm); }
+    sparse_heads(ex);
     const NetLayout &nl = ex->layout;
     for (Step &st : S) st.lane = (nl.side_lo >= 0 && st.layer >= nl.side_lo && st.layer <= nl.side_hi) ? 1 : 0;
 }
@@ -519,9 +556,10 @@
     std::vector<IrbDesc> irb_planned;
     if (plan_layout(ex, irb_planned) || plan_arena(ex) || plan_steps(ex, irb_planned)) return -1;
     rewrite_steps(ex);
-    if (place_constants(ex)) return -1;
+    if (place_constants(ex) || place_sparse(ex)) return -1;
     decide_indirect(ex);
     ex->kernel_count = (int)ex->steps.size();
+    for (const Step &st : ex->steps) if (st.kind == S_CONV && st.conv.sp_list) ex->kernel_count++;
     return 0;
 }
 
@@ -592,7 +630,7 @@
         return ffgpu_launch_front(d, st.irb, in.form, s); }
     case S_YOLO:
         return ffgpu_launch_yolo(st.head, ex->N, ex->in_w, ex->in_h, ex->d_cand, ex->d_cand_key, ex->d_ncand, ex->cand_cap,
-                                 st.flag ? ex->d_ringctr : nullptr, s);
+                                 st.flag ? ex->d_ringctr : nullptr, st.sp_ctr, s);
     case S_NMS:
         return ffgpu_launch_nms(ex->d_cand, ex->d_cand_key, ex->d_ncand, ex->cand_cap, ex->d_full, ex->d_nms_scratch,
                                 ex->d_dets, ex->h_dets_dev, ex->d_ringctr, ex->N, 0.5f, 1, ex->d_prm, s);
@@ -860,7 +898,7 @@
     }
     drop_graphs(ex);
     for (const Step &st : ex->steps) if (st.kind == S_TOCNHW) (void)hipFree(st.out);
-    (void)hipFree(ex->arena); (void)hipFree(ex->d_input); (void)hipFree(ex->d_pack); (void)hipFree(ex->d_cand);
+    (void)hipFree(ex->arena); (void)hipFree(ex->d_input); (void)hipFree(ex->d_pack); (void)hipFree(ex->d_sparse); (void)hipFree(ex->d_cand);
     (void)hipFree(ex->d_cand_key); (void)hipFree(ex->d_ncand); (void)hipFree(ex->d_dets);
     (void)hipFree(ex->d_full); (void)hipFree(ex->d_prm); (void)hipFree(ex->d_nms_scratch); (void)hipFree(ex->d_ftab);
     (void)hipFree(ex->d_merged); (void)hipFree(ex->d_merged_full); (void)hipFree(ex->d_merge_scratch); (void)hipFree(ex->d_mtab);
@@ -1524,6 +1562,10 @@
         if (fl > cap_floats) { ffgpu_set_error("read_layer: buffer too small"); return -1; }
         if (copy_d2h(host_out, ex->last.frames + (size_t)frame * fl, fl * sizeof(float))) return -1;
         return (int)fl;
+    }
+    if (layer >= 0 && layer < ex->net->layer_num && ex->layout.canon[layer] == layer && !ex->layout.readable[layer]) {
+        ffgpu_set_error("read_layer: layer %d is not materialised by this executor (fused away or no tensor)", layer);
+        return -1;
     }
     if (!(ex->flags & FFGPU_KEEP_ALL)) { ffgpu_set_error("read_layer needs an FFGPU_KEEP_ALL executor"); return -1; }
     if (layer < 0 || layer >= ex->net->layer_num || ex->layout.canon[layer] < 0 || !ex->layout.readable[layer]) {
@@ -1754,6 +1796,24 @@
     return ffgpu_launch_conv(d, variant, (hipStream_t)stream);
 }
 
+extern "C" int ffgpu_sparse_head_dev(const float *d_in, const float *d_filt, float *d_out, int batch, int iw, int ih, int ic, int classes, int act,
+                                     float thresh, int *d_list, int *d_count, void *stream)
+{
+    if (!d_in || !d_filt || !d_out || !d_list || !d_count || batch < 1 || iw < 1 || ih < 1 || classes < 1 || classes > 4096) { ffgpu_set_error("sparse_head_dev: bad arguments"); return -1; }
+    ConvDesc d;
+    fill_desc(d, d_in, d_filt, d_out, batch, iw, ih, ic, 1, 0, 1, 1, iw, ih, 3 * (5 + classes), act, 0);
+    d.sp_classes = classes; d.sp_thresh = thresh; d.sp_list = d_list; d.sp_ctr = d_count;
+    return ffgpu_launch_conv(d, FFGPU_K_CONV_X3, (hipStream_t)stream);
+}
+
+extern "C" int ffgpu_sparse_head_launch_text(int batch, int iw, int ih, int ic, int classes, int flags, char *buf, int cap)
+{
+    if (!buf || cap < 1 || batch < 1 || iw < 1 || ih < 1 || ic < 1 || classes < 1) { ffgpu_set_error("sparse_head_launch_text: bad arguments"); return -1; }
+    ConvDesc d;
+    fill_desc(d, nullptr, nullptr, nullptr, batch, iw, ih, ic, 1, 0, 1, 1, iw, ih, 3 * (5 + classes), 0, 0);
+    return ffgpu_conv_sparse_head_line(d, classes, sparse_head_wanted(flags | (knob(K_NO_FUSE) ? FFGPU_NO_FUSE : 0)), buf, (size_t)cap);
+}
+
 extern "C" const char *ffgpu_groupconv_kernel_name(int batch, int iw, int ih, int ic, int groups, int pad,
                                                    int stride, int fs, int fn, int variant)
 {
diff --git a/ffcnn_amd/csrc/ffgpu_kernels.hip b/ffcnn_amd/csrc/ffgpu_kernels.hip
--- a/ffcnn_amd/csrc/ffgpu_kernels.hip
+++ b/ffcnn_amd/csrc/ffgpu_kernels.hip
@@ -208,10 +208,17 @@
 
 #include "ffgpu_block.inc"
 
-__global__ void k_yolo(YoloHead hd, int N, int netw, int neth, BBOX *cand, int *cand_key, int *ncand, int cap, int *ring_ctr)
+__device__ __forceinline__ bool yolo_obj_pass(float bs, float thresh)
+{
+#pragma clang fp contract(off)
+    return !(1.0f / (1.0f + __expf(-bs)) < thresh * 0.999f);
+}
+
+__global__ void k_yolo(YoloHead hd, int N, int netw, int neth, BBOX *cand, int *cand_key, int *ncand, int cap, int *ring_ctr, int *sp_ctr)
 {
 #pragma clang fp contract(off)
     if (ring_ctr && blockIdx.x == 0 && threadIdx.x == 0) *ring_ctr += 1;
+    if (sp_ctr && blockIdx.x == 0 && threadIdx.x == 0) *sp_ctr = 0;
     const int cells = hd.w * hd.h;
     const long total = (long)N * 3 * cells;
     const long gid = (long)blockIdx.x * blockDim.x + threadIdx.x;
@@ -224,7 +231,7 @@
     const long cs = (long)N * cells;
     const float *p = hd.in + (long)k * (5 + hd.classes) * cs + (long)n * cells + cell;
     const float bs = p[4 * cs];
-    const bool pass = gid < total && !(1.0f / (1.0f + __expf(-bs)) < hd.thresh * 0.999f);
+    const bool pass = gid < total && yolo_obj_pass(bs, hd.thresh);
     float cs_best = 0.f;
     int best = 0;
     for (unsigned long long todo = __ballot(pass); todo; todo &= todo - 1) {
@@ -482,10 +489,10 @@
     return 0;
 }
 
-int ffgpu_launch_yolo(const YoloHead &hd, int N, int netw, int neth, BBOX *cand, int *cand_key, int *ncand, int cap, int *ring_ctr, hipStream_t s)
+int ffgpu_launch_yolo(const YoloHead &hd, int N, int netw, int neth, BBOX *cand, int *cand_key, int *ncand, int cap, int *ring_ctr, int *sp_ctr, hipStream_t s)
 {
     const long total = (long)N * 3 * hd.w * hd.h;
-    hipLaunchKernelGGL(k_yolo, dim3((unsigned)((total + 255) / 256)), dim3(256), 0, s, hd, N, netw, neth, cand, cand_key, ncand, cap, ring_ctr);
+    hipLaunchKernelGGL(k_yolo, dim3((unsigned)((total + 255) / 256)), dim3(256), 0, s, hd, N, netw, neth, cand, cand_key, ncand, cap, ring_ctr, sp_ctr);
     LAUNCH_OK("yolo");
     return 0;
 }
diff --git a/ffcnn_amd/csrc/ffgpu_knobs.hpp b/ffcnn_amd/csrc/ffgpu_knobs.hpp
--- a/ffcnn_amd/csrc/ffgpu_knobs.hpp
+++ b/ffcnn_amd/csrc/ffgpu_knobs.hpp
@@ -80,6 +80,7 @@
     X(THIN_PAIR,         "FFGPU_THIN_PAIR",         INT,  1,             TUNING,  "k_irb_thin: 0 keeps FFGPU_CONCURRENT executors off the paired form (two frames per wave, 3 / 4 / 5 columns per lane); read at launch") \
     X(THIN_S2,           "FFGPU_THIN_S2",           INT,  1,             TUNING,  "k_irb_thin_s2: 0 keeps FFGPU_CONCURRENT executors off the streaming form of the stride-2 block 4 -> 24 -> 8 (the planned wave kernel instead); read at launch") \
     X(THIN_S2_BAND,      "FFGPU_THIN_S2_BAND",      INT,  0,             TUNING,  "k_irb_thin_s2: output rows per wave (0: by batch and height, thin_s2_form); read at launch") \
+    X(SPARSE_HEAD,       "FFGPU_SPARSE_HEAD",       INT,  1,             TUNING,  "k_conv_x3: 0 keeps FFGPU_CONCURRENT executors off the sparse form of the pointwise layer in front of a yolo head (a box pass over all pixels, then the class rows of the quads whose objectness can pass; the dense launch instead); read when an executor is created") \
     X(FRONT_BAND,        "FFGPU_FRONT_BAND",       INT,  KNOB_COMPUTED, TUNING,  "k_front: rows per wave; default as FFGPU_THIN_BAND") \
     X(NO_FRONT,          "FFGPU_NO_FRONT",          INT,  0,             PRODUCT, "layers 0-3 as k_conv_first + k_irb_thin instead of k_front") \
     X(FRONT_MIN_PX,      "FFGPU_FRONT_MIN_PX",      INT,  262144,        TUNING,  "k_front: fewest output pixels of the batch") \
diff --git a/include/ffcnn_hip.h b/include/ffcnn_hip.h
--- a/include/ffcnn_hip.h
+++ b/include/ffcnn_hip.h
@@ -166,6 +166,11 @@
 int ffgpu_irb_s2_launch_text(int batch, int iw, int ih, int ic, int ec, int oc, int stride, int act1, int actd, int act2, int res_act,
                              int flags, char *buf, int cap);
 
+int ffgpu_sparse_head_dev(const float *d_in, const float *d_filt, float *d_out, int batch, int iw, int ih, int ic, int classes, int act,
+                          float thresh, int *d_list, int *d_count, void *stream);
+
+int ffgpu_sparse_head_launch_text(int batch, int iw, int ih, int ic, int classes, int flags, char *buf, int cap);
+
 int ffgpu_irb_plan_text(int batch, int iw, int ih, int ic, int ec, int oc, int stride, int act1, int actd, int act2, int res_act,
                         int flags, char *buf, int cap);
 
```
